# JohnGBaker/ptmcmc

Hardware: AMD Instinct MI355X
Metric: ladder-wide MH steps/sec (D=32 Gaussian, 1024 temps) (higher is better)
Workload: dtype f64

## Files before the change

include/ptm_engine.h:

```cpp
#ifndef PTM_ENGINE_H
#define PTM_ENGINE_H

#include <stddef.h>
#include <stdint.h>

#ifdef __cplusplus
extern "C" {
#endif

#define PTM_ABI_VERSION 3

typedef struct ptm_engine ptm_engine;

#define PTM_COUNT_MAX 2147483647

typedef enum {
  PTM_OK = 0,
  PTM_ERR_INVALID = -1,
  PTM_ERR_UNSUPPORTED = -2,
  PTM_ERR_HIP = -3,
  PTM_ERR_NO_DEVICE = -4,
  PTM_ERR_FAR_MOVE = -5,
  PTM_ERR_CALLBACK = -6
} ptm_status;
// ... 94 lines not shown

int ptm_copy_llike(ptm_engine* e, int first_local_rung, int n_rungs, void* dst_dev);
int ptm_llike_device_ptr(ptm_engine* e, void** dev_ptr);
int ptm_exchange_decide(ptm_engine* e, const void* ll_below_dev, const void* ll_above_dev, int halo_rungs, void* send_up_dev,
                        void* send_down_dev);
int ptm_exchange_decide_gathered(ptm_engine* e, const void* ll_all_dev, const void* lp_all_dev, void* send_up_dev, void* send_down_dev);
int ptm_set_shard_map(ptm_engine* e, int n_shards, const int32_t* rung_counts, int halo_rungs);
int ptm_exchange_redo_count(ptm_engine* e, int* n_ladders);
int ptm_exchange_redo(ptm_engine* e, const void* ll_all_dev, const void* lp_all_dev, void* send_up_dev, void* send_down_dev);
int ptm_copy_lprior(ptm_engine* e, int first_local_rung, int n_rungs, void* dst_dev);
int ptm_exchange_finish_and_sweep(ptm_engine* e, const void* recv_from_below_dev, const void* recv_from_above_dev);
int ptm_exchange_install(ptm_engine* e, const void* recv_from_below_dev, const void* recv_from_above_dev);
int ptm_sweep_rungs(ptm_engine* e, int first_local_rung, int n_rungs, int closes_step);
int ptm_exchange_buffer_doubles(ptm_engine* e);
int ptm_exchange_row_capacity(ptm_engine* e);

#define PTM_SHARD_ID_BYTES 128
int ptm_shard_unique_id(void* id_out);
int ptm_shard_init(ptm_engine* e, const void* id, int rank, int world, const int32_t* rung_counts, int halo_rungs);
int ptm_shard_step(ptm_engine* e, int n);
int ptm_shard_finalize(ptm_engine* e);

enum {
  PTM_ARR_LLIKE = 0,
  PTM_ARR_LPRIOR = 1,
  PTM_ARR_LPOST = 2,
  PTM_ARR_NTRIES = 3,
  PTM_ARR_NACCEPT = 4,
  PTM_ARR_LAST_TYPE = 5,
  PTM_ARR_NHIST = 6,
  PTM_ARR_NSIZE = 7,
  PTM_ARR_ROW_LABELS = 8
};
int ptm_get_states(ptm_engine* e, double* X);
int ptm_get_array(ptm_engine* e, int which, void* out);
int ptm_get_swap_counts(ptm_engine* e, int64_t* tries, int64_t* accepts);
int ptm_get_last_swaps(ptm_engine* e, int32_t* pairs, int32_t* accepted);
int ptm_batch_begin(ptm_engine* e);
int ptm_batch_end(ptm_engine* e);
int ptm_restore(ptm_engine* e, const double* X, const double* llike, const int32_t* ntries, const int32_t* naccept,
                const int32_t* last_type, const int64_t* nhist, uint64_t step_count, const int64_t* swap_tries,
                const int64_t* swap_accepts);
int ptm_max_swaps_per_step(ptm_engine* e);
int ptm_get_history(ptm_engine* e, double* X, double* llike, double* lprior, int32_t* meta);
int ptm_get_history_invtemps(ptm_engine* e, double* beta);
int ptm_get_history_chains(ptm_engine* e, int chain_begin, int chain_count, double* X, double* llike, double* lprior, int32_t* meta, double* invtemps);
int ptm_set_history(ptm_engine* e, const double* X, const double* llike, const double* lprior, const int32_t* meta,
                    const double* invtemps);
int ptm_set_map(ptm_engine* e, const double* X, const double* lpost, const double* llike, const double* lprior);
int ptm_get_map(ptm_engine* e, double* X, double* lpost, double* llike, double* lprior);
uint64_t ptm_step_count(ptm_engine* e);

int ptm_timer_start(ptm_engine* e);
int ptm_timer_stop(ptm_engine* e, float* elapsed_ms);
int ptm_get_kernel_times(ptm_engine* e, float* ms, int capacity, int* count);
const char* ptm_sweep_kernel_name(ptm_engine* e);
const char* ptm_step_kernel_name(ptm_engine* e);

int ptm_get_ladder_stats(ptm_engine* e, int64_t out[4]);
int ptm_get_counter_sums(ptm_engine* e, int64_t* ntries_sum, int64_t* naccept_sum);
int ptm_get_prefilter_counts(ptm_engine* e, int64_t out[4]);
typedef struct ptm_calibration {
  double copy_GBs, copy_bytes, copy_ms;
  double f64_fma_TFs, fma_ms, sclk_MHz;
  int32_t compute_units, reserved;
} ptm_calibration;
int ptm_calibrate(ptm_engine* e, ptm_calibration* out);

int ptm_ess_windowed(ptm_engine* e, int rung, int nfeat, int width, int every, int burn, double* ess , int32_t* nwin );
int ptm_ess_report(ptm_engine* e, int rung, int nfeat, int width, int every, double esslimit, double* ess , int32_t* length );
int ptm_ess_series_windowed(int device, const double* series, int64_t n, int nseries, int nfeat, int width, int every, int burn, double* ess, int32_t* nwin);
int ptm_ess_series_report(int device, const double* series, int64_t n, int nseries, int nfeat, int width, int every, double esslimit, double* ess, int32_t* length);
int ptm_ess_last_on_device(ptm_engine* e);

int ptm_log_evidence(ptm_engine* e, int ilen, double* log_evidence , double* up ,
                     double* down , int32_t* count );

enum { PTM_FN_LOG = 0, PTM_FN_EXP = 1, PTM_FN_SIN_0_PI = 2, PTM_FN_COS_HPI = 3, PTM_FN_SQRT = 4, PTM_FN_DIV = 5,
       PTM_FN_SQRT_RAW = 6 };
int ptm_debug_eval(int device, int fn, const double* a, const double* b, double* out, int n);
int ptm_debug_philox(int device, uint64_t seed, int tag, uint32_t stream, uint64_t step, uint32_t block, uint32_t out[4]);
int ptm_debug_boxmuller(int device, const uint32_t* k1, const uint32_t* k2, double* z0, double* z1, int n);
int ptm_debug_sqrt_scan(int device, uint64_t* mismatches);
int ptm_dev_alloc(size_t bytes, void** out);
int ptm_dev_free(void* p);
int ptm_dev_copy(void* dst, const void* src, size_t bytes);
int ptm_debug_evaluate(ptm_engine* e, const double* X, int n, int32_t* valid, double* X_enforced, double* lprior,
                       double* llike);

#ifdef __cplusplus
}
#endif
#endif
```

ptmcmc_amd/csrc/ptm_aux_kernels.hpp:

```cpp
#pragma once
#include "ptm_kernels.hpp"
#include "ptm_decide.hpp"

namespace ptm {

constexpr int PART_CHUNK = 16384;
__global__ __launch_bounds__(1024) void partition_kernel(int W, int rung0, int nchunk, unsigned char* __restrict__ touch,
                                                         unsigned int* __restrict__ nhist, int* __restrict__ cidx, int* __restrict__ ccnt,
                                                         const unsigned short* __restrict__ rowof, const unsigned char* __restrict__ pflag,
                                                         int* __restrict__ pidx, int* __restrict__ pcnt) {
  extern __shared__ int plist[];
  __shared__ int wsum[16];
  __shared__ int sbase, stotal;
  const int rl = rung0 + blockIdx.x / nchunk, ch = blockIdx.x % nchunk;
  const bool pre = pflag && pflag[rl];
  int* const lidx = pre ? pidx : cidx;
  int* const lcnt = pre ? pcnt : ccnt;
  const int w0 = ch * PART_CHUNK + threadIdx.x * 16;
  const size_t c0 = (size_t)rl * W + w0;
  uint4 v = make_uint4(0x01010101u, 0x01010101u, 0x01010101u, 0x01010101u);
  const bool in = w0 < W;
  if (in) v = *reinterpret_cast<const uint4*>(touch + c0);
  const unsigned int word[4] = {v.x, v.y, v.z, v.w};
  int mine = 0;
// ... 243 lines not shown
  double *x, *ll, *lp;
  const double *recv_below, *recv_above;
  int *arr_below, *arr_above;
  int* err;
};
__global__ __launch_bounds__(256) void install_kernel(const Install p) {
  const double* msg = blockIdx.y ? p.recv_above : p.recv_below;
  if (!msg) return;
  int* arr = blockIdx.y ? p.arr_above : p.arr_below;
  int n = *reinterpret_cast<const int*>(msg);
  if (n > p.row_cap) n = p.row_cap;
  const int j = blockIdx.x * 16 + (threadIdx.x >> 4), sub = threadIdx.x & 15;
  if (j >= n) return;
  const int DP = p.DP, RD = DP + ROW_EXTRA;
  const double* row = msg + MSG_HDR + (size_t)j * RD;
  const int w = (int)row[DP + 2];
  const int a = (w >= 0 && w < p.W) ? arr[w] : -1;
  if (a < 0) { atomicOr(p.err, 8); return; }
  for (int col = 2 * sub; col < DP; col += 32)
    *reinterpret_cast<d2_t*>(p.x + (size_t)a * DP + col) = *reinterpret_cast<const d2_t*>(row + col);
  if (sub == 0) { p.ll[a] = row[DP]; p.lp[a] = row[DP + 1]; }
}

__global__ void hist_init_kernel(Hist h, int DP, const double* x, const double* ll, const double* lp, const int* naccept,
                                 const int* ntries, const int* last_type, const double* beta, const double* betaC, int W, int r0) {
  const int c = blockIdx.x * blockDim.x + threadIdx.x;
  if (c >= h.HC) return;
  const size_t o = hist_slot(h, 0, c);
  for (int d = 0; d < DP; ++d) h.x[o * DP + d] = x[(size_t)c * DP + d];
  hist_scalars(h, o, 0, ll[c], lp[c], naccept[c], ntries[c], last_type[c], betaC ? betaC[c] : beta[r0 + c / W]);
}
__global__ void hist_beta_fill_kernel(Hist h, const double* beta, int W, int r0) {
  const size_t i = (size_t)blockIdx.x * blockDim.x + threadIdx.x;
  if (i >= (size_t)h.cap * h.HC) return;
  h.beta[i] = beta[r0 + (int)(i % h.HC) / W];
}

__global__ void map_init_kernel(MapT m, int DP, int W, int r0, const double* beta, const double* x, const double* ll, const double* lp) {
  const int c = blockIdx.x * blockDim.x + threadIdx.x;
  if (c >= m.MC) return;
  m.lpost[c] = -1e200;
  const double t = beta[r0 + c / W] * ll[c];
  if (map_try(m, c, lp[c] + t, ll[c], lp[c]))
    for (int d = 0; d < DP; ++d) m.x[(size_t)c * DP + d] = x[(size_t)c * DP + d];
}

__global__ void debug_eval_kernel(int fn, const double* a, const double* b, double* out, int n) {
  const int i = blockIdx.x * blockDim.x + threadIdx.x;
  if (i >= n) return;
  double r = 0;
  switch (fn) {
    case 0: r = dlog(a[i]); break;
    case 1: r = dexp(a[i]); break;
    case 2: r = dsin_0_pi(a[i]); break;
    case 3: r = dcos_hpi(a[i]); break;
    case 4: r = dsqrt(a[i]); break;
    case 5: r = a[i] / b[i]; break;
    case 6: r = __builtin_sqrt(a[i]); break;
  }
  out[i] = r;
}
__global__ void debug_philox_kernel(uint64_t seed, int tag, uint32_t stream, uint64_t step, uint32_t block, uint32_t* out) {
  const u32x4 o = draw_block(seed, tag, stream, step, block);
  out[0] = o.v0; out[1] = o.v1; out[2] = o.v2; out[3] = o.v3;
}
__global__ void debug_boxmuller_kernel(const uint32_t* k1, const uint32_t* k2, double* z0, double* z1, int n) {
  const int i = blockIdx.x * blockDim.x + threadIdx.x;
  if (i >= n) return;
  boxmuller(k1[i], k2[i], (const double*)BM_TABLE, z0[i], z1[i]);
}
__global__ void debug_sqrt_scan_kernel(unsigned long long* mismatches) {
  const uint32_t tid = blockIdx.x * blockDim.x + threadIdx.x;
  const uint32_t stride = gridDim.x * blockDim.x;
  unsigned long long bad = 0, out = 0;
  for (uint64_t k = tid; k < (1ull << 32); k += stride) {
    const double a = bm_neg2log((uint32_t)k, (const double*)BM_TABLE);
    if (bm_sqrt(a) != dsqrt(a)) bad++;
    if (!(a > 0.0 && a < 64.0)) out++;
  }
  if (bad) atomicAdd(mismatches, bad);
  if (out) atomicAdd(mismatches + 1, out);
}

__global__ __launch_bounds__(256) void calib_copy_kernel(const uint4* __restrict__ src, uint4* __restrict__ dst, size_t n16) {
  const size_t stride = (size_t)gridDim.x * blockDim.x;
  for (size_t i = (size_t)blockIdx.x * blockDim.x + threadIdx.x; i < n16; i += stride) dst[i] = src[i];
}
__global__ __launch_bounds__(256) void counter_sums_kernel(const int* __restrict__ ntries, const int* __restrict__ naccept, size_t n, unsigned long long* __restrict__ out) {
  __shared__ unsigned long long sh[2][4];
  unsigned long long t = 0, a = 0;
  const size_t stride = (size_t)gridDim.x * blockDim.x;
  for (size_t i = (size_t)blockIdx.x * blockDim.x + threadIdx.x; i < n; i += stride) { t += (unsigned long long)(long long)ntries[i]; a += (unsigned long long)(long long)naccept[i]; }
#pragma unroll
  for (int o = 32; o > 0; o >>= 1) { t += __shfl_down(t, o); a += __shfl_down(a, o); }
  if ((threadIdx.x & 63) == 0) { sh[0][threadIdx.x >> 6] = t; sh[1][threadIdx.x >> 6] = a; }
  __syncthreads();
  if (threadIdx.x == 0) {
    atomicAdd(out, sh[0][0] + sh[0][1] + sh[0][2] + sh[0][3]);
    atomicAdd(out + 1, sh[1][0] + sh[1][1] + sh[1][2] + sh[1][3]);
  }
}
__global__ __launch_bounds__(256) void calib_fma_kernel(double* __restrict__ out, long long* __restrict__ clk, int iters) {
  double d[8];
  const double e0 = 1.0 - 1e-9 * (threadIdx.x & 7), e1 = 1e-12 * (1 + (threadIdx.x & 3));
#pragma unroll
  for (int i = 0; i < 8; ++i) d[i] = 1.0 + 1e-3 * (threadIdx.x + i);
  __syncthreads();
  const long long c0 = (long long)__builtin_amdgcn_s_memtime(), r0 = (long long)__builtin_amdgcn_s_memrealtime();
  for (int it = 0; it < iters; ++it) {
#pragma unroll
    for (int i = 0; i < 8; ++i) asm volatile("v_fma_f64 %0, %0, %1, %2" : "+v"(d[i]) : "v"(e0), "v"(e1));
  }
  const long long c1 = (long long)__builtin_amdgcn_s_memtime(), r1 = (long long)__builtin_amdgcn_s_memrealtime();
  double r = 0.0;
#pragma unroll
  for (int i = 0; i < 8; ++i) r += d[i];
  if (r == 12345.678) out[0] = r;
  if (threadIdx.x == 0) { clk[2 * blockIdx.x] = c1 - c0; clk[2 * blockIdx.x + 1] = r1 - r0; }
}

}
```

ptmcmc_amd/csrc/ptm_box_prefilter.hpp:

```cpp
#pragma once
#include "ptm_kernels.hpp"
#include "ptm_sweep_plan.hpp"

namespace ptm {

#ifndef PTM_BP_ROWS_AHEAD
#define PTM_BP_ROWS_AHEAD 0
#endif

struct BoxPre {
  int W, Nt, r0, w_off;
  int rung0, nrung;
  int labelled;
  uint64_t seed, step;
  const double* x;
  const double *ll, *lp;
  const double* beta;
  const double* prop_tiles;
  const double* box_row;
  int* ntries;
  const int *pidx, *pcnt;
  int *cidx, *ccnt;
  unsigned long long* counts;
};
// ... 72 lines not shown
  PrefilterSlice sl[EA + 1] = {};
  int m[EA + 1] = {};
  BpRows R[2] = {};
#pragma unroll
  for (int k = 0; k < EA; ++k) { sl[k] = slice_of((int)blockIdx.x + k * G); m[k] = load_entry(sl[k]); }
  if (RA) load_rows(sl[0], m[0], R[0]);
  uint64_t pbits = 0;
  int pmine = 0, pbase = 0;
  size_t plbase = 0;
  auto flush = [&]() {
    if (pbits == 0) return;
    const int base = __builtin_amdgcn_readfirstlane(pbase);
    if ((pbits >> l) & 1ull) p.cidx[plbase + base + __builtin_popcountll(pbits & ((1ull << l) - 1ull))] = pmine;
    pbits = 0;
  };
#define PTM_BP_ARRIVED() __builtin_amdgcn_s_waitcnt(0x0F70)
  PTM_BP_ARRIVED();
  unsigned int seen = 0, settled = 0;
  for (int tile = blockIdx.x; tile < ntiles; tile += G) {
    sl[EA] = slice_of(tile + EA * G);
    m[EA] = load_entry(sl[EA]);
    if (RA) load_rows(sl[1], m[1], R[1]);
    else load_rows(sl[0], m[0], R[0]);
    PTM_BP_STAGE();
    const PrefilterSlice s = sl[0];
    const int mine = m[0], nact = s.nact;
    const int rl = p.rung0 + s.r, rg = p.r0 + rl;
    const size_t lbase = (size_t)rl * p.W;
    const BpRows& T = R[0];
    uint64_t inbox = 0;
    if (nact) {
      const bp_d2 lo0 = box[0], lo1 = box[4], hi0 = box[16], hi1 = box[20];
#pragma unroll
      for (int g = 0; g < 4; ++g) {
        const int wk = __shfl(mine, 16 * g + j, 64) & wmask;
        const uint32_t stream = (uint32_t)(wk + p.w_off) * (uint32_t)p.Nt + (uint32_t)rg;
        const u32x4 o = draw_block(p.seed, TAG_MH, stream, p.step, (uint32_t)(1 + q));
        double z[4];
        boxmuller(o.v0, o.v1, L.bm, z[0], z[1]);
        boxmuller(o.v2, o.v3, L.bm, z[2], z[3]);
        bp_d4 acc = bp_d4{0.0, 0.0, 0.0, 0.0};
#pragma unroll
        for (int k = 0; k < 4; ++k) acc = __builtin_amdgcn_mfma_f64_16x16x4f64(T.ta[k], z[k], acc, 0, 0, 0);
        const double x0 = T.v0[g].x + acc[0], x1 = T.v0[g].y + acc[1], x2 = T.v1[g].x + acc[2], x3 = T.v1[g].y + acc[3];
        const bool ok = !(x0 < lo0.x) & !(x0 > hi0.x) & !(x1 < lo0.y) & !(x1 > hi0.y) & !(x2 < lo1.x) & !(x2 > hi1.x) & !(x3 < lo1.y) & !(x3 > hi1.y);
        uint64_t b = __builtin_amdgcn_ballot_w64(ok);
        b &= b >> 32;
        b &= b >> 16;
        inbox |= (b & 0xFFFFull) << (16 * g);
      }
    }
    PTM_BP_STAGE();
    PTM_BP_ARRIVED();
    if (nact) {
      const int c = (int)lbase + (mine & wmask);
      const double cur_lpost = T.lp + T.beta * T.ll;
      const bool live = l < nact;
      const bool finite = __builtin_fabs(cur_lpost) < __builtin_inf();
      const bool settle = live && finite && ((inbox >> l) & 1ull) == 0;
      const bool keep = live && !settle;
      const uint64_t kbits = __builtin_amdgcn_ballot_w64(keep);
      const int nk = __builtin_popcountll(kbits);
      flush();
      if (settle) (void)__hip_atomic_fetch_add(&p.ntries[c], 1, __ATOMIC_RELAXED, __HIP_MEMORY_SCOPE_AGENT);
      if (nk) {
        pbits = kbits; pmine = mine; plbase = lbase;
        const int rlv = __builtin_amdgcn_mov_dpp(rl, 0xE4, 0xF, 0xF, true);
        if (l == 0) pbase = atomicAdd(&p.ccnt[rlv], nk);
      }
      seen += (unsigned int)nact;
      settled += (unsigned int)(nact - nk);
    }
#pragma unroll
    for (int k = 0; k < EA; ++k) { sl[k] = sl[k + 1]; m[k] = m[k + 1]; }
    if (RA) R[0] = R[1];
  }
  flush();
  if (l == 0 && seen) {
    atomicAdd(p.counts, (unsigned long long)seen);
    if (settled) atomicAdd(p.counts + 1, (unsigned long long)settled);
  }
}

}
```

ptmcmc_amd/csrc/ptm_device_math.hpp:

```cpp
#pragma once
#include <hip/hip_runtime.h>
#include <stdint.h>

#include "ptm_lds_layout.hpp"

namespace ptm {

struct u32x4 { uint32_t v0, v1, v2, v3; };
#ifndef PTM_PHILOX_ROUNDS
#define PTM_PHILOX_ROUNDS 10
#endif

struct philox_state { uint32_t c0, c1, c2, c3, k0, k1; };
__device__ __forceinline__ void philox_round(philox_state& s) {
  const uint64_t p0 = (uint64_t)0xD2511F53u * s.c0;
  const uint64_t p1 = (uint64_t)0xCD9E8D57u * s.c2;
  const uint32_t n0 = (uint32_t)(p1 >> 32) ^ s.c1 ^ s.k0;
  const uint32_t n1 = (uint32_t)p1;
  const uint32_t n2 = (uint32_t)(p0 >> 32) ^ s.c3 ^ s.k1;
  const uint32_t n3 = (uint32_t)p0;
  s.c0 = n0; s.c1 = n1; s.c2 = n2; s.c3 = n3;
  s.k0 += 0x9E3779B9u; s.k1 += 0xBB67AE85u;
}
__device__ __forceinline__ u32x4 philox4x32_10(uint32_t c0, uint32_t c1, uint32_t c2, uint32_t c3, uint32_t k0,
// ... 162 lines not shown
}
__device__ __forceinline__ double draw_copolar(double u, double lo, double hi) {
  const double sl = dsin_hpi(lo), sh = dsin_hpi(hi);
  const double y = sl + u * (sh - sl);
  double a = lo, b = hi;
#pragma unroll 1
  for (int k = 0; k < 64; ++k) {
    const double m = 0.5 * (a + b);
    if (dsin_hpi(m) < y) a = m; else b = m;
  }
  return 0.5 * (a + b);
}
__device__ __forceinline__ double draw_log(double u, double lo, double hi) {
  const double l0 = dlog(lo);
  return dexp(u * (dlog(hi) - l0) + l0);
}

__device__ __forceinline__ double dsqrt(double a) {
  const double g = __builtin_sqrt(a);
  const double r = __builtin_fma(-g, g, a);
  const double gn = __longlong_as_double(__double_as_longlong(g) + (r > 0.0 ? 1 : -1));
  const double t = __builtin_fma(-g, gn, a);
  const bool move = (r > 0.0) ? (t > 0.0) : ((r < 0.0) ? (t <= 0.0) : false);
  const bool ok = (a > 0.0) && (a < __builtin_inf());
  return (ok && move) ? gn : g;
}

#include "ptm_tables.inc"
__device__ __attribute__((aligned(16))) const double BM_TABLE[BM_TABLE_DOUBLES] = {PTM_BMTAB_VALUES, PTM_TRIGTAB_VALUES};

typedef double bm_d2 __attribute__((ext_vector_type(2)));

template <class Tab>
__device__ __forceinline__ double bm_neg2log(uint32_t k, Tab tab) {
  const double M2LN2_HI = -2.0 * 6.93147180369123816490e-01, M2LN2_LO = -2.0 * 1.90821492927058770002e-10;
  const double x = (double)k + 0.5;
  const uint64_t b = (uint64_t)__double_as_longlong(x);
  const uint32_t hi = (uint32_t)(b >> 32);
  const uint32_t idx = (hi >> 12) & 255u;
  const int e = (int)(hi >> 20) - (1023 + 32) + (idx >= (uint32_t)PTM_BMTAB_SPLIT ? 1 : 0);
  const double m = __longlong_as_double((long long)((b & 0x000FFFFFFFFFFFFFull) | 0x3FF0000000000000ull));
  const bm_d2 ra = *reinterpret_cast<const bm_d2*>(tab + 2 * idx);
  const double t = __builtin_fma(m, ra.x, -1.0);
  double q = 1.0 / 3.0;
  q = __builtin_fma(q, t, -0.4);
  q = __builtin_fma(q, t, 0.5);
  q = __builtin_fma(q, t, -2.0 / 3.0);
  q = __builtin_fma(q, t, 1.0);
  const double l = __builtin_fma(t * t, q, -2.0 * t);
  const double dk = (double)e;
  return __builtin_fma(dk, M2LN2_HI, ra.y) + __builtin_fma(dk, M2LN2_LO, l);
}

__device__ __forceinline__ double bm_sqrt(double a) {
  const double y = __builtin_amdgcn_rsq(a);
  double g = a * y;
  double h = 0.5 * y;
  const double r = __builtin_fma(-h, g, 0.5);
  g = __builtin_fma(g, r, g);
  h = __builtin_fma(h, r, h);
  const double d = __builtin_fma(-g, g, a);
  return __builtin_fma(d, h, g);
}

template <class Tab>
__device__ __forceinline__ void boxmuller_finish(double r, uint32_t k2, Tab tab, double& z0, double& z1) {
  const uint32_t idx = (k2 >> 21) & 1023u;
  const bm_d2 sc = *reinterpret_cast<const bm_d2*>(tab + 512 + 2 * idx);
  const double d = __builtin_fma((double)((int)(k2 & 0x1FFFFFu) - (1 << 20)), 1.4629180792671596e-09, 0.5 * 1.4629180792671596e-09);
  const double d2 = d * d;
  const double sd = __builtin_fma(d * d2, __builtin_fma(d2, 1.0 / 120.0, -1.0 / 6.0), d);
  const double cm1 = d2 * __builtin_fma(d2, 1.0 / 24.0, -0.5);
  const double sn = __builtin_fma(sc.y, sd, sc.x * cm1) + sc.x;
  const double cs = __builtin_fma(-sc.x, sd, sc.y * cm1) + sc.y;
  r = __longlong_as_double(__double_as_longlong(r) ^ ((long long)(k2 >> 31) << 63));
  z0 = r * cs;
  z1 = r * sn;
}
template <typename Tab>
__device__ __forceinline__ void boxmuller(uint32_t k1, uint32_t k2, Tab tab, double& z0, double& z1) {
  boxmuller_finish(bm_sqrt(bm_neg2log(k1, tab)), k2, tab, z0, z1);
}

__device__ __forceinline__ double fmod_det(double x, double w) {
  const double q = __builtin_trunc(x / w);
  double r = __builtin_fma(-q, w, x);
  if (x >= 0.0) { if (r < 0.0) r += w; else if (r >= w) r -= w; }
  else          { if (r > 0.0) r -= w; else if (r <= -w) r += w; }
  return r;
}

}
```

ptmcmc_amd/csrc/ptm_engine.hip:

```cpp
#include <hip/hip_runtime.h>

#include <algorithm>
#include <cmath>
#include <cstddef>
#include <cstdarg>
#include <cstdio>
#include <cstring>
#include <functional>
#include <memory>
#include <string>
#include <vector>

#include "../../include/ptm_engine.h"
#include "ptm_aux_kernels.hpp"
#include "ptm_box_prefilter.hpp"
#include "ptm_count_limit.hpp"
#include "ptm_de_mfma_kernel.hpp"
#include "ptm_devlike_kernels.hpp"
#include "ptm_ess_kernels.hpp"
#include "ptm_evidence_kernels.hpp"
#include "ptm_launch.hpp"
#include "ptm_shard_rccl.hpp"

using namespace ptm;
// ... 14 lines not shown
    if (_e != hipSuccess) return fail(PTM_ERR_HIP, "%s failed: %s (%s:%d)", #x, hipGetErrorString(_e), __FILE__, __LINE__); \
  } while (0)

template <class T>
struct PinnedAlloc {
  typedef T value_type;
  PinnedAlloc() {}
  template <class U> PinnedAlloc(const PinnedAlloc<U>&) {}
  T* allocate(size_t n) {
    void* p = nullptr;
    if (hipHostMalloc(&p, n * sizeof(T), hipHostMallocMapped | hipHostMallocCoherent) != hipSuccess) throw std::bad_alloc();
    return (T*)p;
  }
  void deallocate(T* p, size_t) { (void)hipHostFree(p); }
  template <class U> bool operator==(const PinnedAlloc<U>&) const { return true; }
  template <class U> bool operator!=(const PinnedAlloc<U>&) const { return false; }
};
template <class T> using pinned_vector = std::vector<T, PinnedAlloc<T>>;

struct ptm_engine {
  ptm_config cfg;
  int D = 0, DP = 0, Nt = 0, r0 = 0, nloc = 0, W = 0, Nc = 0, ms = 0;
  int device = 0;
  hipStream_t stream = nullptr;
  bool own_stream = false;
  uint64_t step = 0;
  double *xdev = nullptr, *ll = nullptr, *lp = nullptr;
  int *ntries = nullptr, *naccept = nullptr, *last_type = nullptr, *err = nullptr;
  int *arr_below = nullptr, *arr_above = nullptr;
  int *mv_src = nullptr, *mv_dst = nullptr, *mv_n = nullptr;
  unsigned int* nhist = nullptr;
  long long* swap_cnt = nullptr;
  unsigned char* touch = nullptr;
  Hist hist = {0, 0, 0, nullptr, nullptr, nullptr, nullptr, nullptr};
  MapT map = {0, 0, nullptr, nullptr, nullptr, nullptr};
  int* swap_log = nullptr;
  int log_head = 0, log_pending = 0;
  int row_cap = 0;
  int *blo = nullptr, *bhi = nullptr, *ptype = nullptr;
  double *bmin = nullptr, *bmax = nullptr, *plo = nullptr, *phi = nullptr, *pcoef = nullptr;
  double *P2 = nullptr, *mean = nullptr, *beta = nullptr, *prop = nullptr, *prop_tiles = nullptr, *P2_tiles = nullptr, *box_row = nullptr, *onedfrac = nullptr, *mix = nullptr;
  int mix_K = 0;
  bool de_on = false;
  ptm_de_params de = {0, 0, 0, 0};
  int de_init_extra = 0;
  double *de_init = nullptr, *de_hast = nullptr;
  int* de_type = nullptr;
  bool ada_on = false;
  ptm_adaptive_set ada = {0, -1, 0, 0, 0};
  double *ada_leaf = nullptr, *ada_dbl = nullptr;
  int* ada_int = nullptr;
  int prior_member = -1;
  std::vector<char> set_neg;
  double evolve_rate = 0, evolve_cut = -1;
  double *beta_w = nullptr, *betaC = nullptr, *beta_add = nullptr;
  bool betaC_stale = false;
  int has_bounds = 0, origin_valid = 1, all_uniform = 1, has_mean = 0, have_target = 0, have_ladder = 0,
      have_prop = 0, have_state = 0, prop_kind = KIND_DIAG, prop_stride = 0, any_oned = 0, bounds_box = 1;
  double lprior_const = 0, like0 = 0, thresh = 0;
  bool lp_is_const = false;
  std::vector<double> h_beta;
  std::vector<int> h_ptype;
  std::vector<double> h_plo, h_phi;
  ptm_loglike_batch_fn cb = nullptr;
  void* cb_user = nullptr;
  ptm_logprior_batch_fn prior_cb = nullptr;
  void* prior_user = nullptr;
  ptm_propose_batch_fn pcb = nullptr;
  ptm_proposal_result_fn pres = nullptr;
  void* pcb_user = nullptr;
  ptm_loglike_device_fn dfn = nullptr;
  void* dfn_user = nullptr;
  double *dl_x = nullptr, *dl_ll = nullptr;
  bool dl_own_x = false, dl_own_ll = false;
  int32_t* dl_count = nullptr;
  int *dl_rows = nullptr, *dl_chunks = nullptr;
  double *dl_xprop = nullptr, *dl_lprior_new = nullptr, *dl_llike_new = nullptr, *dl_best = nullptr;
  unsigned char* dl_gate = nullptr;
  int *cidx = nullptr, *ccnt = nullptr;
  int *pidx = nullptr, *pcnt = nullptr;
  unsigned char *pf_flag = nullptr, *h_pf_flag = nullptr;
  unsigned long long* pf_counts = nullptr;
  std::vector<double> pf_sigma;
  bool pf_dirty = true;
  int pf_flagged = 0, pf_grid = 0;
  bool touched = false;
  bool compact_step = false;
  unsigned short* rowof = nullptr;
  bool rows_labelled = false;
  bool label_step = false;
  ShardComm* shard = nullptr;
  int* shard_ends = nullptr;
  int nshards = 0, halo_nominal = 0;
  int* redo_flag = nullptr;
  long long redo_total = 0;
  double *pub_x = nullptr, *pub_ll = nullptr, *pub_lp = nullptr;
  int *lad_flags = nullptr, *lad_ctl = nullptr;
  long long* lad_prof = nullptr;
  int lad_capacity[2][32] = {{-1, -1, -1, -1, -1, -1, -1, -1, -1, -1, -1, -1, -1, -1, -1, -1, -1, -1, -1, -1, -1, -1, -1, -1, -1, -1, -1, -1, -1, -1, -1, -1},
                             {-1, -1, -1, -1, -1, -1, -1, -1, -1, -1, -1, -1, -1, -1, -1, -1, -1, -1, -1, -1, -1, -1, -1, -1, -1, -1, -1, -1, -1, -1, -1, -1}};
  long long ladder_launches = 0, ladder_whole_steps = 0;
  struct LadLaunch { int seq; uint64_t step_before; int nsteps; int log_head_before; };
  std::vector<LadLaunch> lad_log;
  int lad_deferred = 0;
  int lad_seq = 0;
  bool lad_disabled = false;
  long long ladder_fallbacks = 0;
  hipEvent_t lad_event = nullptr;
  unsigned int nhist_pending = 0;
  CountHorizon horizon;
  bool step_booked = false;
  int steps_prepaid = 0;
  double* hastings = nullptr;
  int* htype = nullptr;
  unsigned char *hvalid = nullptr, *acc_out = nullptr;
  pinned_vector<double> h_rows, h_hast;
  pinned_vector<int> h_type;
  pinned_vector<unsigned char> h_valid, h_touch, h_acc;
  std::vector<double> p_xcur, p_xprop, p_hast;
  std::vector<int32_t> p_rung, p_walker, p_type, p_valid, p_acc;
  std::vector<size_t> p_pick;
  double *xprop = nullptr, *lprior_new = nullptr, *llike_new = nullptr;
  pinned_vector<unsigned char> fetch_arena;
  size_t fetch_used = 0;
  int fetch_depth = 0;
  std::vector<std::function<void()>> fetch_after;
  std::vector<std::shared_ptr<std::vector<unsigned char>>> fetch_big;
  std::vector<std::pair<unsigned char*, size_t>> host_blocks;
  bool shared_handover = false, hist_on_host = false;
  unsigned char* gate = nullptr;
  pinned_vector<double> h_xprop, h_llnew;
  std::vector<double> h_batch, h_llbatch;
  unsigned char* h_gate = nullptr;
  unsigned long long *sums = nullptr, *h_sums = nullptr;
  void* ess_ws = nullptr;
  size_t ess_ws_bytes = 0;
  int ess_on_device = 0;
  hipEvent_t t0 = nullptr, t1 = nullptr;
  std::vector<hipEvent_t> kev;
  size_t kev_used = 0;
  std::string kname;
};

#include <mutex>
static std::mutex g_lad_mutex;
static ptm_engine* g_lad_last = nullptr;

static int round_dp(int D) {
  if (D <= 4) return 4;
  if (D <= 8) return 8;
  if (D <= 16) return 16;
  if (D <= 32) return 32;
  if (D <= 64) return 64;
  if (D <= 128) return 128;
  if (D <= 256) return 256;
  if (D <= 512) return 512;
  return 1024;
}

template <class T>
static int dalloc(T** p, size_t n) {
  HIPCHK(hipMalloc((void**)p, (n ? n : 1) * sizeof(T)));
  return PTM_OK;
}
static hipError_t copy_unless_shared(void* dst, const void* src, size_t bytes, hipMemcpyKind kind, hipStream_t s) {
  if (dst == src) return hipSuccess;
// ... 162 lines not shown
  e->all_uniform = 0;
  HIPCHK(hipEventCreate(&e->t0));
  HIPCHK(hipEventCreate(&e->t1));
  HIPCHK(hipStreamSynchronize(e->stream));
  return PTM_OK;
}

template <class T>
static int halloc(ptm_engine* e, T** p, size_t n) {
  void* h = nullptr;
  const size_t bytes = (n ? n : 1) * sizeof(T);
  HIPCHK(hipHostMalloc(&h, bytes, hipHostMallocMapped | hipHostMallocCoherent));
  e->host_blocks.push_back(std::make_pair((unsigned char*)h, bytes));
  *p = (T*)h;
  return PTM_OK;
}

static const size_t FETCH_ARENA = (size_t)4 << 20;
static int fetch_flush(ptm_engine* e) {
  HIPCHK(hipStreamSynchronize(e->stream));
  for (auto& f : e->fetch_after) f();
  e->fetch_after.clear(); e->fetch_big.clear(); e->fetch_used = 0;
  return PTM_OK;
}
static int fetch_raw(ptm_engine* e, const void* dev, size_t bytes, const unsigned char** staged) {
  for (const auto& b : e->host_blocks)
    if ((const unsigned char*)dev >= b.first && (const unsigned char*)dev < b.first + b.second) {
      *staged = (const unsigned char*)dev;
      return PTM_OK;
    }
  if (e->fetch_arena.empty()) e->fetch_arena.resize(FETCH_ARENA);
  const size_t need = (bytes + 63) & ~(size_t)63;
  if (need > FETCH_ARENA / 2 || e->fetch_used + need > FETCH_ARENA) {
    auto buf = std::make_shared<std::vector<unsigned char>>(bytes);
    HIPCHK(hipStreamSynchronize(e->stream));
    HIPCHK(hipMemcpy(buf->data(), dev, bytes, hipMemcpyDeviceToHost));
    e->fetch_big.push_back(buf);
    *staged = buf->data();
    return PTM_OK;
  }
  unsigned char* at = e->fetch_arena.data() + e->fetch_used;
  HIPCHK(hipMemcpyAsync(at, dev, bytes, hipMemcpyDeviceToHost, e->stream));
  e->fetch_used += need;
  *staged = at;
  return PTM_OK;
}
static int fetch(ptm_engine* e, const void* dev, size_t bytes, const unsigned char** staged) {
  const int rc = fetch_raw(e, dev, bytes, staged);
  if (rc) { e->fetch_after.clear(); e->fetch_big.clear(); e->fetch_used = 0; }
  return rc;
}
static int fetch_done(ptm_engine* e) { return e->fetch_depth > 0 ? PTM_OK : fetch_flush(e); }
#define SETTLE(e) do { if (e) { const int _rc = ladder_settle(e); if (_rc) return _rc; } } while (0)
#define NO_BATCH(e, name) do { if ((e) && (e)->fetch_depth > 0) return fail(PTM_ERR_INVALID, name " between ptm_batch_begin and ptm_batch_end (only reads go there)"); } while (0)
#define FETCH(ptr, dev, bytes) do { int _rc = fetch(e, (dev), (bytes), &(ptr)); if (_rc) return _rc; } while (0)

extern "C" int ptm_batch_begin(ptm_engine* e) {
  SETTLE(e);
  if (!e) return fail(PTM_ERR_INVALID, "null engine");
  e->fetch_depth++;
  return PTM_OK;
}
extern "C" int ptm_batch_end(ptm_engine* e) {
  if (!e) return fail(PTM_ERR_INVALID, "null engine");
  if (e->fetch_depth <= 0) return fail(PTM_ERR_INVALID, "ptm_batch_end without ptm_batch_begin");
  if (--e->fetch_depth > 0) return PTM_OK;
  return fetch_flush(e);
}

extern "C" int ptm_engine_destroy(ptm_engine* e) {
  if (!e) return PTM_OK;
  (void)ptm_shard_finalize(e);
  (void)hipStreamSynchronize(e->stream);
  {
    std::lock_guard<std::mutex> lock(g_lad_mutex);
    if (g_lad_last == e) g_lad_last = nullptr;
  }
  if (e->lad_event) (void)hipEventDestroy(e->lad_event);
  if (e->shared_handover) e->xprop = e->llike_new = nullptr, e->hastings = nullptr, e->htype = nullptr, e->hvalid = e->acc_out = nullptr;
  if (e->hist_on_host) e->hist.x = e->hist.ll = e->hist.lp = e->hist.beta = nullptr, e->hist.meta = nullptr;
  for (auto& b : e->host_blocks) (void)hipHostFree(b.first);
  void* ptrs[] = {e->xdev, e->rowof, e->ll, e->lp, e->ntries, e->naccept, e->last_type, e->arr_below, e->arr_above, e->mv_src, e->mv_dst, e->mv_n,
                  e->err, e->nhist, e->swap_cnt, e->touch, e->swap_log, e->hist.x, e->hist.ll, e->hist.lp, e->hist.meta, e->map.lpost, e->map.ll, e->map.lp, e->map.x, e->blo,
                  e->bhi, e->ptype, e->bmin, e->bmax, e->plo, e->phi, e->pcoef, e->P2, e->mean, e->beta, e->prop, e->prop_tiles, e->P2_tiles, e->box_row, e->onedfrac, e->mix, e->beta_w, e->betaC, e->beta_add, e->hist.beta, e->xprop, e->lprior_new, e->llike_new, e->hastings, e->htype, e->hvalid, e->acc_out, e->cidx, e->ccnt, e->pidx, e->pcnt, e->pf_flag, e->pf_counts,
                  e->pub_x, e->lad_flags, e->lad_prof, e->shard_ends, e->redo_flag, e->sums, e->de_init, e->de_hast, e->de_type,
                  e->ada_leaf, e->ada_dbl, e->ada_int, e->dl_own_x ? e->dl_x : nullptr, e->dl_own_ll ? e->dl_ll : nullptr, e->dl_count, e->dl_rows, e->dl_chunks, e->dl_xprop,
                  e->dl_lprior_new, e->dl_llike_new, e->dl_best, e->ess_ws};
  for (void* p : ptrs)
    if (p) (void)hipFree(p);
  if (e->h_sums) (void)hipHostFree(e->h_sums);
  if (e->h_pf_flag) (void)hipHostFree(e->h_pf_flag);
  for (hipEvent_t ev : e->kev) (void)hipEventDestroy(ev);
  if (e->t0) (void)hipEventDestroy(e->t0);
  if (e->t1) (void)hipEventDestroy(e->t1);
  if (e->own_stream) (void)hipStreamDestroy(e->stream);
  delete e;
  return PTM_OK;
}

extern "C" int ptm_set_bounds(ptm_engine* e, const int32_t* lo, const int32_t* hi, const double* xmin, const double* xmax) {
  SETTLE(e);
  if (!e || !lo || !hi || !xmin || !xmax) return fail(PTM_ERR_INVALID, "null argument");
  int rc;
  const int D = e->D;
  e->has_bounds = 0;
  e->bounds_box = 1;
  for (int d = 0; d < D; ++d) {
    if (lo[d] < 0 || lo[d] > 3 || hi[d] < 0 || hi[d] > 3) return fail(PTM_ERR_INVALID, "bad boundary type in dimension %d", d);
    if (lo[d] != PTM_BOUND_OPEN || hi[d] != PTM_BOUND_OPEN) e->has_bounds = 1;
    if ((lo[d] != PTM_BOUND_OPEN && lo[d] != PTM_BOUND_LIMIT) || (hi[d] != PTM_BOUND_OPEN && hi[d] != PTM_BOUND_LIMIT)) e->bounds_box = 0;
  }
  e->origin_valid = 1;
  for (int d = 0; d < D; ++d) {
    const bool lw = lo[d] == PTM_BOUND_WRAP, hw = hi[d] == PTM_BOUND_WRAP;
    if (lw != hw) { e->origin_valid = 0; break; }
    if (lw) { if (xmax[d] - xmin[d] <= 0) { e->origin_valid = 0; break; } continue; }
    if (lo[d] == PTM_BOUND_REFLECT && hi[d] == PTM_BOUND_REFLECT) { if (xmax[d] - xmin[d] <= 0) { e->origin_valid = 0; break; } continue; }
    double z = 0.0;
    if (lo[d] == PTM_BOUND_REFLECT && z < xmin[d]) z = xmin[d] + (xmin[d] - z);
    else if (hi[d] == PTM_BOUND_REFLECT && z > xmax[d]) z = xmax[d] - (z - xmax[d]);
    if (lo[d] == PTM_BOUND_LIMIT && z < xmin[d]) { e->origin_valid = 0; break; }
    if (hi[d] == PTM_BOUND_LIMIT && z > xmax[d]) { e->origin_valid = 0; break; }
  }
  if ((rc = upload(e->blo, lo, D, e->stream)) || (rc = upload(e->bhi, hi, D, e->stream)) ||
      (rc = upload(e->bmin, xmin, D, e->stream)) || (rc = upload(e->bmax, xmax, D, e->stream)))
    return rc;
  return PTM_OK;
}

static inline size_t host_row_pos(size_t DP, size_t d);
extern "C" int ptm_set_prior(ptm_engine* e, const int32_t* types, const double* c, const double* h) {
  SETTLE(e);
  if (!e || !types || !c || !h) return fail(PTM_ERR_INVALID, "null argument");
  const int D = e->D;
  std::vector<double> lo(D), hi(D), coef(D);
  std::vector<int> ty(D);
  e->all_uniform = 1;
  double prod = 1;
  for (int d = 0; d < D; ++d) {
    ty[d] = types[d];
    switch (types[d]) {
      case PTM_PRIOR_FLAT: lo[d] = -INFINITY; hi[d] = INFINITY; coef[d] = 1; e->all_uniform = 0; break;
      case PTM_PRIOR_UNIFORM: lo[d] = c[d] - h[d]; hi[d] = c[d] + h[d]; coef[d] = 1 / (hi[d] - lo[d]); prod *= coef[d]; break;
      case PTM_PRIOR_GAUSSIAN: lo[d] = c[d]; hi[d] = h[d]; coef[d] = 0; e->all_uniform = 0; break;
      case PTM_PRIOR_POLAR: {
        double a = c[d] - h[d], b = c[d] + h[d];
        lo[d] = a; hi[d] = b;
        if (a < 0) a = 0;
        if (b > M_PI) b = M_PI;
        coef[d] = -std::cos(b) + std::cos(a);
        e->all_uniform = 0;
        break;
      }
      case PTM_PRIOR_COPOLAR: {
        double a = c[d] - h[d], b = c[d] + h[d];
        lo[d] = a; hi[d] = b;
        if (a < -M_PI / 2) a = -M_PI / 2;
        if (b > M_PI / 2) b = M_PI / 2;
        coef[d] = std::sin(b) - std::sin(a);
        e->all_uniform = 0;
        break;
      }
      case PTM_PRIOR_LOG:
        if (c[d] <= 0 || h[d] <= 1) return fail(PTM_ERR_INVALID, "log prior needs center>0 and halfwidth>1 (dimension %d)", d);
        lo[d] = c[d] / h[d]; hi[d] = c[d] * h[d]; coef[d] = std::log(hi[d]) - std::log(lo[d]);
        e->all_uniform = 0;
        break;
      default: return fail(PTM_ERR_INVALID, "unknown prior type %d in dimension %d", types[d], d);
    }
  }
  e->lprior_const = std::log(prod);
  e->pf_dirty = true;
  e->lp_is_const = false;
  for (int d = 0; d < D; ++d) { e->h_ptype[d] = ty[d]; e->h_plo[d] = lo[d]; e->h_phi[d] = hi[d]; }
// ... 240 lines not shown

extern "C" int ptm_set_invtemps(ptm_engine* e, const double* beta) {
  SETTLE(e);
  NO_BATCH(e, "ptm_set_invtemps");
  if (!e || !beta) return fail(PTM_ERR_INVALID, "null argument");
  if (!e->beta_w) return fail(PTM_ERR_INVALID, "per-ladder temperatures exist only once the ladders evolve (ptm_set_evolve_temps)");
  HIPCHK(hipStreamSynchronize(e->stream));
  HIPCHK(hipMemcpy(e->beta_w, beta, (size_t)e->W * e->Nt * 8, hipMemcpyHostToDevice));
  return launch_beta_transpose(e);
}

extern "C" int ptm_set_proposals(ptm_engine* e, int kind, const double* factors, const double* one_d_frac) {
  SETTLE(e);
  if (!e || !factors) return fail(PTM_ERR_INVALID, "null argument");
  const int D = e->D, DP = e->DP, nloc = e->nloc;
  int stride;
  std::vector<double> packed;
  if (kind == PTM_PROP_DIAG) {
    stride = DP;
    packed.assign((size_t)nloc * stride, 0.0);
    for (int r = 0; r < nloc; ++r)
      for (int d = 0; d < D; ++d) packed[(size_t)r * stride + d] = factors[(size_t)r * D + d];
  } else if (kind == PTM_PROP_DENSE || kind == PTM_PROP_LOWER) {
    stride = DP * DP;
    packed.assign((size_t)nloc * stride, 0.0);
    for (int r = 0; r < nloc; ++r)
      for (int i = 0; i < D; ++i)
        for (int j = 0; j < D; ++j) packed[(size_t)r * stride + (size_t)j * DP + i] = factors[(size_t)r * D * D + (size_t)i * D + j];
    if (kind == PTM_PROP_LOWER)
      for (int r = 0; r < nloc; ++r)
        for (int i = 0; i < D; ++i)
          for (int j = i + 1; j < D; ++j)
            if (factors[(size_t)r * D * D + (size_t)i * D + j] != 0.0)
              return fail(PTM_ERR_INVALID, "PTM_PROP_LOWER factor of local rung %d has a non-zero above the diagonal", r);
  } else {
    return fail(PTM_ERR_INVALID, "unknown proposal kind %d", kind);
  }
  if (e->prop) { HIPCHK(hipStreamSynchronize(e->stream)); HIPCHK(hipFree(e->prop)); e->prop = nullptr; }
  if (e->prop_tiles) { HIPCHK(hipFree(e->prop_tiles)); e->prop_tiles = nullptr; }
  int rc;
  if ((rc = dalloc(&e->prop, packed.size())) || (rc = upload(e->prop, packed.data(), packed.size(), e->stream))) return rc;
  if (DP == 32) {
    std::vector<double> tiles((size_t)nloc * 16 * 64, 0.0);
    for (int r = 0; r < nloc; ++r)
      for (int t = 0; t < 16; ++t) {
        const int rt = t & 1, sl = (t >> 1) & 3, hb = t >> 3;
        for (int k = 0; k < 4; ++k)
          for (int i = 0; i < 16; ++i) {
            const int row = 16 * rt + i, col = 16 * hb + 4 * k + sl;
            if (row < D && col < D)
              tiles[((size_t)r * 16 + t) * 64 + 16 * k + i] =
                  kind == PTM_PROP_DIAG ? (row == col ? factors[(size_t)r * D + row] : 0.0) : factors[(size_t)r * D * D + (size_t)row * D + col];
          }
      }
    if ((rc = dalloc(&e->prop_tiles, tiles.size())) || (rc = upload(e->prop_tiles, tiles.data(), tiles.size(), e->stream))) return rc;
  }
  if (DP == 64 || DP == 128) {
    const int NT = DP / 16, ntile = NT * NT * 4;
    std::vector<double> tiles((size_t)nloc * ntile * 64, 0.0);
    for (int r = 0; r < nloc; ++r)
      for (int t = 0; t < ntile; ++t) {
        const int rt = t % NT, sl = (t / NT) & 3, hb = t / (4 * NT);
        for (int k = 0; k < 4; ++k)
          for (int i = 0; i < 16; ++i) {
            const int row = 16 * rt + i, col = 16 * hb + 4 * k + sl;
            if (row < D && col < D)
              tiles[((size_t)r * ntile + t) * 64 + 16 * k + i] =
                  kind == PTM_PROP_DIAG ? (row == col ? factors[(size_t)r * D + row] : 0.0) : factors[(size_t)r * D * D + (size_t)row * D + col];
          }
      }
    if ((rc = dalloc(&e->prop_tiles, tiles.size())) || (rc = upload(e->prop_tiles, tiles.data(), tiles.size(), e->stream))) return rc;
  }
  std::vector<double> f(nloc, 0.0);
  e->any_oned = 0;
  if (one_d_frac)
    for (int r = 0; r < nloc; ++r) {
      if (one_d_frac[r] < 0 || one_d_frac[r] > 1) return fail(PTM_ERR_INVALID, "oneDfrac must be in [0,1]");
      f[r] = one_d_frac[r];
      if (f[r] > 0) e->any_oned = 1;
    }
  if ((rc = upload(e->onedfrac, f.data(), (size_t)nloc, e->stream))) return rc;
  e->prop_kind = kind; e->prop_stride = stride; e->have_prop = 1;
  e->pf_sigma.assign((size_t)nloc * PREFILTER_DIMS, 0.0);
  for (int r = 0; r < nloc; ++r) prefilter_sigmas(kind == PTM_PROP_DIAG, factors + (size_t)r * (kind == PTM_PROP_DIAG ? D : D * D), D, &e->pf_sigma[(size_t)r * PREFILTER_DIMS]);
  e->pf_dirty = true;
  return PTM_OK;
}

static int ada_off(ptm_engine* e) {
  e->ada_on = false;
  if (!e->ada_leaf && !e->ada_dbl && !e->ada_int) return PTM_OK;
  HIPCHK(hipStreamSynchronize(e->stream));
  if (e->ada_leaf) HIPCHK(hipFree(e->ada_leaf));
  if (e->ada_dbl) HIPCHK(hipFree(e->ada_dbl));
  if (e->ada_int) HIPCHK(hipFree(e->ada_int));
  e->ada_leaf = e->ada_dbl = nullptr;
  e->ada_int = nullptr;
  return PTM_OK;
}

extern "C" int ptm_set_proposal_mixture(ptm_engine* e, int K, const double* cum_shares, const double* scales, const double* one_d_fracs) {
  SETTLE(e);
  if (!e) return fail(PTM_ERR_INVALID, "null engine");
  if (!e->have_prop) return fail(PTM_ERR_INVALID, "set the base proposals first (ptm_set_proposals)");
  if (K < 0 || K > 64) return fail(PTM_ERR_INVALID, "mixture size must be in 0..64");
  if (e->mix) { HIPCHK(hipStreamSynchronize(e->stream)); HIPCHK(hipFree(e->mix)); e->mix = nullptr; }
  e->mix_K = 0;
  e->prior_member = -1; e->set_neg.clear();
  { const int rc = ada_off(e); if (rc) return rc; }
  if (K == 0) return PTM_OK;
  if (!cum_shares || !scales || !one_d_fracs) return fail(PTM_ERR_INVALID, "null argument");
  const int nloc = e->nloc;
  std::vector<double> t((size_t)nloc * K * 3);
  int oned = 0;
  for (int r = 0; r < nloc; ++r)
    for (int k = 0; k < K; ++k) {
      const size_t i = (size_t)r * K + k;
      if (k > 0 && cum_shares[i] < cum_shares[i - 1]) return fail(PTM_ERR_INVALID, "cumulative shares must not decrease (rung %d)", r);
      if (one_d_fracs[i] < 0 || one_d_fracs[i] > 1) return fail(PTM_ERR_INVALID, "oneDfrac must be in [0,1]");
      t[3 * i] = cum_shares[i]; t[3 * i + 1] = scales[i]; t[3 * i + 2] = one_d_fracs[i];
      if (one_d_fracs[i] > 0) oned = 1;
    }
  int rc;
  if ((rc = dalloc(&e->mix, t.size())) || (rc = upload(e->mix, t.data(), t.size(), e->stream))) return rc;
  e->mix_K = K;
  e->set_neg.assign((size_t)K, 0);
  for (int r = 0; r < nloc; ++r)
    for (int k = 0; k < K; ++k)
      if (scales[(size_t)r * K + k] < 0) e->set_neg[k] = 1;
  if (oned) e->any_oned = 1;
  return PTM_OK;
}

static int ada_check_state(const ptm_adaptive_set& a, size_t Nc, const double* w, const double* th, const int32_t* bits, const int32_t* cnt) {
  if (!w || !th || !bits || !cnt) return fail(PTM_ERR_INVALID, "null argument");
  const int L = a.K + a.K_inner;
  for (size_t c = 0; c < Nc; ++c)
    for (int b = 0; b < 2; ++b) {
      const int first = b ? a.K : 0, n = b ? a.K_inner : a.K;
      const int32_t bv = bits[c * 2 + b], cv = cnt[c * 2 + b];
      if (bv < 0 || (n < 31 && bv >= (1 << n)) || cv < 0)
        return fail(PTM_ERR_INVALID, "adaptive set: repeat bits name members of the set only and outcome counts are >= 0 (chain %zu)", c);
      if (n == 0) continue;
      double sum = 0.0, prev = 0.0;
      for (int k = 0; k < n; ++k) {
        const double wk = w[c * L + first + k], tk = th[c * L + first + k];
        if (!std::isfinite(wk) || wk < 0) return fail(PTM_ERR_INVALID, "adaptive set: weights must be finite and >= 0 (chain %zu)", c);
        if (!(tk >= prev && tk <= 1.0)) return fail(PTM_ERR_INVALID, "adaptive set: thresholds must not decrease and lie in [0, 1] (chain %zu)", c);
        sum += wk;
        prev = tk;
      }
      if (!(sum > 0)) return fail(PTM_ERR_INVALID, "adaptive set: the weights of a set must have a positive sum (chain %zu)", c);
      if (prev != 1.0) return fail(PTM_ERR_INVALID, "adaptive set: the last threshold of a set must be exactly 1 (chain %zu)", c);
    }
  return PTM_OK;
}
static void ada_to_soa(size_t Nc, int L, const double* w, const double* th, const int32_t* bits, const int32_t* cnt, std::vector<double>& dbl, std::vector<int>& in) {
  dbl.assign(2 * (size_t)L * Nc, 0.0);
  in.assign(4 * Nc, 0);
  for (size_t c = 0; c < Nc; ++c) {
    for (int k = 0; k < L; ++k) { dbl[(size_t)k * Nc + c] = w[c * L + k]; dbl[((size_t)L + k) * Nc + c] = th[c * L + k]; }
    for (int b = 0; b < 2; ++b) { in[(size_t)b * Nc + c] = bits[c * 2 + b]; in[(size_t)(2 + b) * Nc + c] = cnt[c * 2 + b]; }
  }
}

extern "C" int ptm_set_proposal_adaptive(ptm_engine* e, const ptm_adaptive_set* a, const double* scales, const double* one_d_fracs, const double* weights,
                                         const double* thresholds, const int32_t* repeat_bits, const int32_t* outcomes) {
// ... 124 lines not shown
  SETTLE(e);
  if (!e) return fail(PTM_ERR_INVALID, "null engine");
  NO_BATCH(e, "ptm_set_proposal_de");
  HIPCHK(hipStreamSynchronize(e->stream));
  if (e->de_init) { HIPCHK(hipFree(e->de_init)); e->de_init = nullptr; }
  e->de_on = false; e->de_init_extra = 0;
  if (!q) return PTM_OK;
  if (e->DP > 128) return fail(PTM_ERR_UNSUPPORTED, "differential evolution on the device is built for up to 128 dimensions; above, draw it on the host (ptm_set_proposal_callback)");
  if (e->nloc != e->Nt)
    return fail(PTM_ERR_UNSUPPORTED, "differential evolution draws from EVERY rung's saved history, and a rung shard cannot record its top rung's: the row that "
                                     "rung holds between two exchanges of one step sits in the shard above (error bit 16).  Split the population by walkers "
                                     "(whole ladders per GPU: walker_begin) or draw on the host (ptm_set_proposal_callback)");
  if (e->hist.rungs != e->nloc || e->hist.cap < 2)
    return fail(PTM_ERR_INVALID, "differential evolution draws from every rung's saved history: create the engine with history_rungs = rung_count and a "
                                 "history_capacity that holds every row of the run");
  if (e->pcb) return fail(PTM_ERR_INVALID, "host-side proposals are set (ptm_set_proposal_callback): they replace every device proposal");
  if (!(q->snooker >= 0 && q->snooker <= 1) || !(q->gamma_one_frac >= 0 && q->gamma_one_frac <= 1) || !(q->reduce_gamma > 0) ||
      !(q->ignore_frac >= 0 && q->ignore_frac < 1) || n_init_extra < 0 || (n_init_extra > 0 && !init_rows))
    return fail(PTM_ERR_INVALID, "differential evolution: snooker and gamma_one_frac in [0, 1], reduce_gamma > 0, ignore_frac in [0, 1), init rows given");
  int rc;
  if (n_init_extra > 0) {
    const size_t Nc = e->Nc, D = e->D, DP = e->DP;
    std::vector<double> img((size_t)n_init_extra * Nc * DP, 0.0);
    for (size_t k = 0; k < (size_t)n_init_extra; ++k)
      for (size_t c = 0; c < Nc; ++c)
        for (size_t d = 0; d < D; ++d) img[(k * Nc + c) * DP + host_row_pos(DP, d)] = init_rows[(k * Nc + c) * D + d];
    if ((rc = dalloc(&e->de_init, img.size()))) return rc;
    HIPCHK(hipMemcpy(e->de_init, img.data(), img.size() * 8, hipMemcpyHostToDevice));
  }
  if (!e->de_hast && ((rc = dalloc(&e->de_hast, (size_t)e->Nc)) || (rc = dalloc(&e->de_type, (size_t)e->Nc)))) return rc;
  e->de = *q;
  e->de_init_extra = n_init_extra;
  e->de_on = true;
  return PTM_OK;
}

extern "C" int ptm_set_proposal_rung(ptm_engine* e, int local_rung, const double* factor, double one_d_frac) {
  SETTLE(e);
  if (!e || !factor) return fail(PTM_ERR_INVALID, "null argument");
  if (!e->have_prop) return fail(PTM_ERR_INVALID, "set all proposals first (ptm_set_proposals)");
  if (local_rung < 0 || local_rung >= e->nloc) return fail(PTM_ERR_INVALID, "rung out of the shard");
  const int D = e->D, DP = e->DP, kind = e->prop_kind == KIND_DIAG ? PTM_PROP_DIAG : (e->prop_kind == KIND_LOWER ? PTM_PROP_LOWER : PTM_PROP_DENSE);
  std::vector<double> packed((size_t)e->prop_stride, 0.0);
  if (kind == PTM_PROP_DIAG) {
    for (int d = 0; d < D; ++d) packed[d] = factor[d];
  } else {
    for (int i = 0; i < D; ++i)
      for (int j = 0; j < D; ++j) {
        if (kind == PTM_PROP_LOWER && j > i && factor[(size_t)i * D + j] != 0.0)
          return fail(PTM_ERR_INVALID, "PTM_PROP_LOWER factor has a non-zero above the diagonal");
        packed[(size_t)j * DP + i] = factor[(size_t)i * D + j];
      }
  }
  int rc;
  if ((rc = upload(e->prop + (size_t)local_rung * e->prop_stride, packed.data(), packed.size(), e->stream))) return rc;
  if (DP == 32) {
    std::vector<double> tiles(16 * 64, 0.0);
    for (int t = 0; t < 16; ++t) {
      const int rt = t & 1, sl = (t >> 1) & 3, hb = t >> 3;
      for (int k = 0; k < 4; ++k)
        for (int i = 0; i < 16; ++i) {
          const int row = 16 * rt + i, col = 16 * hb + 4 * k + sl;
          if (row < D && col < D)
            tiles[(size_t)t * 64 + 16 * k + i] = kind == PTM_PROP_DIAG ? (row == col ? factor[row] : 0.0) : factor[(size_t)row * D + col];
        }
    }
    if ((rc = upload(e->prop_tiles + (size_t)local_rung * 16 * 64, tiles.data(), tiles.size(), e->stream))) return rc;
  }
  if (DP == 64 || DP == 128) {
    const int NT = DP / 16, ntile = NT * NT * 4;
    std::vector<double> tiles((size_t)ntile * 64, 0.0);
    for (int t = 0; t < ntile; ++t) {
      const int rt = t % NT, sl = (t / NT) & 3, hb = t / (4 * NT);
      for (int k = 0; k < 4; ++k)
        for (int i = 0; i < 16; ++i) {
          const int row = 16 * rt + i, col = 16 * hb + 4 * k + sl;
          if (row < D && col < D)
            tiles[(size_t)t * 64 + 16 * k + i] = kind == PTM_PROP_DIAG ? (row == col ? factor[row] : 0.0) : factor[(size_t)row * D + col];
        }
    }
    if ((rc = upload(e->prop_tiles + (size_t)local_rung * ntile * 64, tiles.data(), tiles.size(), e->stream))) return rc;
  }
  prefilter_sigmas(kind == PTM_PROP_DIAG, factor, D, &e->pf_sigma[(size_t)local_rung * PREFILTER_DIMS]);
  e->pf_dirty = true;
  if (one_d_frac >= 0) {
    if (one_d_frac > 1) return fail(PTM_ERR_INVALID, "oneDfrac must be in [0,1]");
    if ((rc = upload(e->onedfrac + local_rung, &one_d_frac, 1, e->stream))) return rc;
    if (one_d_frac > 0) e->any_oned = 1;
  }
  return PTM_OK;
}

static Dev make_dev(ptm_engine* e, bool labelled = false) {
  Dev p;
  memset(&p, 0, sizeof p);
  p.D = e->D; p.DP = e->DP; p.Nt = e->Nt; p.r0 = e->r0; p.nloc = e->nloc; p.W = e->W; p.Nc = e->Nc; p.w_off = e->cfg.walker_begin;
  p.seed = e->cfg.seed; p.step = e->step; p.add_every_n = e->cfg.add_every_n; p.min_prior = e->cfg.min_prior;
  p.has_bounds = e->has_bounds; p.origin_valid = e->origin_valid; p.bounds_box = e->bounds_box;
  p.blo = e->blo; p.bhi = e->bhi; p.bmin = e->bmin; p.bmax = e->bmax;
  p.all_uniform = e->all_uniform; p.lprior_const = e->lprior_const;
  p.ptype = e->ptype; p.plo = e->plo; p.phi = e->phi; p.pcoef = e->pcoef;
  p.P2 = e->P2; p.mean = e->mean; p.has_mean = e->has_mean; p.like0 = e->like0;
  p.beta = e->beta; p.prop = e->prop; p.prop_tiles = e->prop_tiles; p.P2_tiles = e->P2_tiles; p.box_row = e->box_row; p.onedfrac = e->onedfrac; p.prop_stride = e->prop_stride; p.any_oned = e->any_oned;
  p.mix_K = e->mix_K; p.mix = e->mix;
  p.de_on = e->de_on ? 1 : 0; p.de_init_extra = e->de_init_extra; p.de_init = e->de_init; p.de_hast = e->de_hast; p.de_type = e->de_type;
  p.de_snooker = e->de.snooker; p.de_gamma_one = e->de.gamma_one_frac; p.de_gamma_div = e->de.reduce_gamma; p.de_ignore = e->de.ignore_frac;
  p.de_gamma_std = e->de_on ? 1.68 / std::sqrt((double)e->D) / e->de.reduce_gamma : 0.0;
  p.prior_k = e->prior_member + 1;
  p.betaC = e->betaC; p.beta_add = e->beta_add; p.beta_w = e->beta_w;
  p.x = labelled ? e->xdev : xrows(e); p.ll = e->ll; p.lp = e->lp;
  p.ntries = e->ntries; p.naccept = e->naccept; p.last_type = e->last_type; p.nhist = e->nhist;
  p.touch = e->touch; p.err = e->err;
  p.hist = e->hist;
  p.map = e->map;
  p.c_begin = 0; p.c_end = e->Nc;
  p.host_prop = e->pcb ? 1 : 0; p.hastings = e->hastings; p.htype = e->htype; p.hvalid = e->hvalid; p.acc_out = e->acc_out;
  return p;
}

static AdaArgs make_ada(const ptm_engine* e) {
  AdaArgs a;
  memset(&a, 0, sizeof a);
  if (!e->ada_on) return a;
  const size_t L = (size_t)e->ada.K + e->ada.K_inner, Nc = e->Nc;
  a.K = e->ada.K; a.nested = e->ada.nested; a.Ki = e->ada.K_inner; a.rate = e->ada.rate; a.rate_in = e->ada.rate_inner;
  a.leaf = e->ada_leaf; a.w = e->ada_dbl; a.th = e->ada_dbl + L * Nc; a.bits = e->ada_int; a.cnt = e->ada_int + 2 * Nc;
  return a;
}

const DpLaunch* ptm::dp_launch(int DP) {
  switch (DP) {
    case 4: return &dp_launch_4;
    case 8: return &dp_launch_8;
    case 16: return &dp_launch_16;
    case 32: return &dp_launch_32;
    case 64: return &dp_launch_64;
    case 128: return &dp_launch_128;
    case 256: return &dp_launch_256;
    case 512: return &dp_launch_512;
    case 1024: return &dp_launch_1024;
  }
  return nullptr;
}

static inline bool user_like(const ptm_engine* e) { return e->cb != nullptr || e->dfn != nullptr; }

static SweepFacts sweep_facts(const ptm_engine* e, long long chains, bool touched) {
  SweepFacts f;
  memset(&f, 0, sizeof f);
  f.DP = e->DP; f.W = e->W; f.chains = chains; f.nloc = e->nloc;
  f.kind = e->prop_kind == PTM_PROP_DIAG ? PLAN_DIAG : (e->prop_kind == PTM_PROP_LOWER ? PLAN_LOWER : PLAN_DENSE);
  f.has_bounds = e->has_bounds; f.bounds_box = e->bounds_box; f.all_uniform = e->all_uniform; f.has_mean = e->has_mean; f.any_oned = e->any_oned;
  f.mix_K = e->mix_K;
  f.evolving = e->betaC != nullptr; f.tracked = e->hist.rungs || e->map.rungs;
  f.user_like = user_like(e); f.host_prop = e->pcb != nullptr; f.ada = e->ada_on;
  f.de = e->de_on || e->prior_member >= 0;
  f.mode = f.user_like ? 1 : 0;
  f.touched = touched;
  f.prior_draw = e->prior_member >= 0; f.history = e->hist.rungs > 0 && e->hist.rungs == e->nloc;
  return f;
}
static SweepPlan sweep_plan(const ptm_engine* e, long long chains, bool touched) { return plan_sweep(sweep_facts(e, chains, touched), sweep_env()); }
static SweepPlan step_sweep_plan(const ptm_engine* e) { return sweep_plan(e, e->Nc, true); }
static bool de_mfma_sweep(const ptm_engine* e, long long chains) { return e->de_on && de_mfma_applies(sweep_facts(e, chains, true), sweep_env()); }

static bool lean_ev_sweeps(const ptm_engine* e) { return reads_ladder_major_beta(step_sweep_plan(e)); }
// ... 96 lines not shown
  NO_BATCH(e, "ptm_set_target_device");
  if (e->prior_cb) return fail(PTM_ERR_UNSUPPORTED, "a host-evaluated prior with a device likelihood is not built (ptm_set_prior_callback)");
  if (e->pcb) return fail(PTM_ERR_UNSUPPORTED, "host-side proposals with a device likelihood are not built (ptm_set_proposal_callback)");
  if (e->nloc != e->Nt) return fail(PTM_ERR_UNSUPPORTED, "a device likelihood on a rung shard is not built: split such a population by walkers");
  const size_t Nc = e->Nc, D = e->D, DP = e->DP;
  int rc;
  if (!e->dl_count &&
      ((rc = dalloc(&e->dl_count, 1)) || (rc = dalloc(&e->dl_rows, Nc)) || (rc = dalloc(&e->dl_chunks, (Nc + DL_CHUNK - 1) / DL_CHUNK)) ||
       (rc = dalloc(&e->dl_xprop, Nc * DP)) || (rc = dalloc(&e->dl_gate, Nc)) || (rc = dalloc(&e->dl_lprior_new, Nc)) ||
       (rc = dalloc(&e->dl_llike_new, Nc)) || (rc = dalloc(&e->dl_best, D + 1))))
    return rc;
  if (x_batch_dev) {
    if (e->dl_own_x && e->dl_x) { HIPCHK(hipStreamSynchronize(e->stream)); (void)hipFree(e->dl_x); }
    e->dl_x = x_batch_dev; e->dl_own_x = false;
  } else if (!e->dl_own_x) {
    e->dl_x = nullptr;
    if ((rc = dalloc(&e->dl_x, Nc * D))) return rc;
    e->dl_own_x = true;
  }
  if (llike_batch_dev) {
    if (e->dl_own_ll && e->dl_ll) { HIPCHK(hipStreamSynchronize(e->stream)); (void)hipFree(e->dl_ll); }
    e->dl_ll = llike_batch_dev; e->dl_own_ll = false;
  } else if (!e->dl_own_ll) {
    e->dl_ll = nullptr;
    if ((rc = dalloc(&e->dl_ll, Nc))) return rc;
    e->dl_own_ll = true;
  }
  HIPCHK(hipMemsetAsync(e->dl_gate, 0, Nc, e->stream));
  if ((rc = devlike_reset_best(e))) return rc;
  e->dfn = fn; e->dfn_user = user;
  e->cb = nullptr;
  e->have_target = 1;
  return PTM_OK;
}

extern "C" int ptm_target_device_rows(ptm_engine* e) {
  if (!e) return fail(PTM_ERR_INVALID, "null engine");
  return e->Nc;
}

extern "C" int ptm_get_best_evaluated(ptm_engine* e, double* lpost, double* x) {
  if (!e || !lpost) return fail(PTM_ERR_INVALID, "null argument");
  SETTLE(e);
  NO_BATCH(e, "ptm_get_best_evaluated");
  if (!e->dl_best) return fail(PTM_ERR_INVALID, "no device likelihood set (ptm_set_target_device)");
  std::vector<double> b((size_t)e->D + 1);
  HIPCHK(hipMemcpyAsync(b.data(), e->dl_best, b.size() * 8, hipMemcpyDeviceToHost, e->stream));
  HIPCHK(hipStreamSynchronize(e->stream));
  *lpost = b[0];
  if (x) memcpy(x, b.data() + 1, (size_t)e->D * 8);
  return PTM_OK;
}

static int devlike_debug(ptm_engine* e, const double* X, int n, double* llike) {
  const size_t Nc = e->Nc, D = e->D;
  std::vector<double> rows(Nc * D);
  for (size_t k0 = 0; k0 < (size_t)n; k0 += Nc) {
    const size_t m = std::min(Nc, (size_t)n - k0);
    for (size_t k = 0; k < Nc; ++k) memcpy(&rows[k * D], X + (k0 + (k < m ? k : 0)) * D, D * 8);
    const int32_t cnt = (int32_t)m;
    HIPCHK(hipMemcpyAsync(e->dl_x, rows.data(), Nc * D * 8, hipMemcpyHostToDevice, e->stream));
    HIPCHK(hipMemcpyAsync(e->dl_count, &cnt, 4, hipMemcpyHostToDevice, e->stream));
    e->dfn(e->dfn_user, (void*)e->stream, (int)Nc, (int)D, e->dl_x, e->dl_count, e->dl_ll);
    HIPCHK(hipMemcpyAsync(llike + k0, e->dl_ll, m * 8, hipMemcpyDeviceToHost, e->stream));
    HIPCHK(hipStreamSynchronize(e->stream));
  }
  return PTM_OK;
}

#define NO_DEVLIKE(e, name) do { if ((e) && (e)->dfn) return fail(PTM_ERR_UNSUPPORTED, name " with a device likelihood is not built (rung-sharded steps)"); } while (0)

static int prefilter_flags(ptm_engine* e) {
  const int nd = e->D < PREFILTER_DIMS ? e->D : PREFILTER_DIMS;
  double width[PREFILTER_DIMS];
  for (int d = 0; d < nd; ++d) width[d] = e->h_phi[d] - e->h_plo[d];
  if (!e->h_pf_flag) HIPCHK(hipHostMalloc((void**)&e->h_pf_flag, (size_t)e->nloc, hipHostMallocDefault));
  unsigned char* fl = e->h_pf_flag;
  e->pf_flagged = 0;
  for (int r = 0; r < e->nloc; ++r) {
    fl[r] = (e->pf_sigma.size() == (size_t)e->nloc * PREFILTER_DIMS && prefilter_flag(&e->pf_sigma[(size_t)r * PREFILTER_DIMS], width, nd, sweep_env().prefilter)) ? 1 : 0;
    e->pf_flagged += fl[r];
  }
  HIPCHK(hipMemcpyAsync(e->pf_flag, fl, (size_t)e->nloc, hipMemcpyHostToDevice, e->stream));
  e->pf_dirty = false;
  return PTM_OK;
}

static int launch_sweep(ptm_engine* e, int rung0 = 0, int nr = -1, bool last = true) {
  const bool labelled = e->label_step;
  e->label_step = false;
  Dev p = make_dev(e, labelled);
  if (nr < 0) nr = e->nloc - rung0;
  if (rung0 < 0 || nr < 0 || rung0 + nr > e->nloc) return fail(PTM_ERR_INVALID, "rung range out of the shard");
  p.c_begin = rung0 * e->W; p.c_end = (rung0 + nr) * e->W;
  if ((user_like(e) || e->pcb) && (rung0 != 0 || nr != e->nloc)) return fail(PTM_ERR_UNSUPPORTED, "partial sweeps with a user likelihood (host or device) or host-side proposals are not built");
  auto close_step = [&]() {
    e->step += 1; e->touched = false; e->step_booked = false;
    if (e->compact_step) { e->nhist_pending += 1; e->compact_step = false; }
  };
  if (nr == 0) { if (last) close_step(); return PTM_OK; }
  hipEvent_t ev0 = nullptr, ev1 = nullptr;
  if (e->cfg.time_kernels) {
    if (e->kev_used + 2 > e->kev.size()) {
      for (int k = 0; k < 2; ++k) { hipEvent_t ev; HIPCHK(hipEventCreate(&ev)); e->kev.push_back(ev); }
    }
    ev0 = e->kev[e->kev_used]; ev1 = e->kev[e->kev_used + 1];
    e->kev_used += 2;
  }
  const SweepPlan plan = sweep_plan(e, p.c_end - p.c_begin, e->touched);
  if (e->betaC_stale && !reads_ladder_major_beta(plan)) { int rc = ensure_betaC(e); if (rc) return rc; }
  const bool compact = plan.compacted;
  if (labelled && !(compact && rung0 == 0 && nr == e->nloc)) return fail(PTM_ERR_HIP, "internal: a labelled exchange phase without its compacted sweep");
  if (!compact) { int rc = flush_nhist(e); if (rc) return rc; }
  if (compact) {
    if (!e->cidx) { int rc; if ((rc = dalloc(&e->cidx, (size_t)e->Nc)) || (rc = dalloc(&e->ccnt, (size_t)e->nloc))) return rc; }
    HIPCHK(hipMemsetAsync(e->ccnt + rung0, 0, (size_t)nr * sizeof(int), e->stream));
    bool pre = plan.prefilter;
    if (pre) {
      if (!e->pidx) {
        int rc;
        if ((rc = dalloc(&e->pidx, (size_t)e->Nc)) || (rc = dalloc(&e->pcnt, (size_t)e->nloc)) || (rc = dalloc(&e->pf_flag, (size_t)e->nloc)) || (rc = dalloc(&e->pf_counts, 2))) return rc;
        HIPCHK(hipMemsetAsync(e->pf_counts, 0, 16, e->stream));
        e->pf_dirty = true;
      }
      if (e->pf_dirty) { int rc = prefilter_flags(e); if (rc) return rc; }
      pre = e->pf_flagged > 0;
      if (pre) HIPCHK(hipMemsetAsync(e->pcnt + rung0, 0, (size_t)nr * sizeof(int), e->stream));
    }
    const int nchunk = (e->W + PART_CHUNK - 1) / PART_CHUNK;
    hipLaunchKernelGGL(partition_kernel, dim3((unsigned)((size_t)nr * nchunk)), dim3(1024), (size_t)PART_CHUNK * sizeof(int), e->stream, e->W, rung0, nchunk, e->touch, e->nhist,
                       e->cidx, e->ccnt, labelled ? (const unsigned short*)e->rowof : nullptr, pre ? (const unsigned char*)e->pf_flag : nullptr, e->pidx, e->pcnt);
    e->compact_step = true;
    HIPCHK(hipGetLastError());
    if (pre) {
      BoxPre b;
      memset(&b, 0, sizeof b);
      b.W = e->W; b.Nt = e->Nt; b.r0 = e->r0; b.w_off = e->cfg.walker_begin; b.rung0 = rung0; b.nrung = nr; b.labelled = labelled ? 1 : 0;
      b.seed = e->cfg.seed; b.step = e->step;
      b.x = p.x; b.ll = e->ll; b.lp = e->lp; b.beta = e->beta; b.prop_tiles = e->prop_tiles; b.box_row = e->box_row; b.ntries = e->ntries;
      b.pidx = e->pidx; b.pcnt = e->pcnt; b.cidx = e->cidx; b.ccnt = e->ccnt; b.counts = e->pf_counts;
      const size_t lds = BoxPreLds(nullptr, nr).bytes;
      if (!e->pf_grid) {
        int per_cu = 0, dev = 0;
        hipDeviceProp_t pr;
        if (hipOccupancyMaxActiveBlocksPerMultiprocessor(&per_cu, (const void*)box_prefilter_kernel, 256, BoxPreLds(nullptr, e->nloc).bytes) != hipSuccess || per_cu <= 0) { (void)hipGetLastError(); per_cu = 2; }
        HIPCHK(hipGetDevice(&dev));
        HIPCHK(hipGetDeviceProperties(&pr, dev));
        e->pf_grid = per_cu * (pr.multiProcessorCount > 0 ? pr.multiProcessorCount : 256);
        const int cap = sweep_env().prefilter_grid;
        if (cap > 0 && cap < e->pf_grid) e->pf_grid = cap;
      }
      const long long tiles = (long long)nr * ((e->W + 255) / 256);
      hipLaunchKernelGGL(box_prefilter_kernel, dim3((unsigned)(tiles < e->pf_grid ? tiles : e->pf_grid)), dim3(256), lds, e->stream, b);
      HIPCHK(hipGetLastError());
    }
    p.cidx = e->cidx; p.ccnt = e->ccnt; p.cidx_slot = labelled ? 1 : 0;
  }
  if (ev0) HIPCHK(hipEventRecord(ev0, e->stream));
  const AdaArgs ada = make_ada(e);
  const DpLaunch* dl = dp_launch(e->DP);
  if (!dl) return fail(PTM_ERR_UNSUPPORTED, "dim > 1024 is not built");
  const bool de_mfma = de_mfma_sweep(e, p.c_end - p.c_begin);
  if (de_mfma && (compact || plan.family == FAM_MFMA32)) return fail(PTM_ERR_HIP, "internal: differential evolution on the matrix cores beside a matrix-core plan");
  auto launch = [&](const Dev& q) {
    if (de_mfma) return launch_de_mfma32(q, e->prop_kind == PTM_PROP_DENSE ? KIND_DENSE : KIND_LOWER, e->betaC != nullptr, e->stream);
    return dl->sweep(q, plan, e->stream, ada);
  };

  size_t npick = 0;
  if (e->pcb) {
    const size_t Nc = e->Nc, D = e->D, DP = e->DP;
    HIPCHK(hipMemcpyAsync(e->h_rows.data(), xrows(e), Nc * DP * 8, hipMemcpyDeviceToHost, e->stream));
    HIPCHK(hipMemcpyAsync(e->h_touch.data(), e->touch, Nc, hipMemcpyDeviceToHost, e->stream));
    HIPCHK(hipStreamSynchronize(e->stream));
    e->p_pick.clear();
    for (size_t c = 0; c < Nc; ++c)
      if (!e->h_touch[c]) e->p_pick.push_back(c);
    npick = e->p_pick.size();
    e->p_xcur.resize(npick * D); e->p_xprop.assign(npick * D, 0.0); e->p_hast.assign(npick, 0.0);
    e->p_rung.resize(npick); e->p_walker.resize(npick); e->p_type.assign(npick, 0); e->p_valid.assign(npick, 1);
    for (size_t k = 0; k < npick; ++k) {
      const size_t c = e->p_pick[k];
      for (size_t d = 0; d < D; ++d) e->p_xcur[k * D + d] = e->h_rows[c * DP + host_row_pos(DP, d)];
      e->p_rung[k] = e->r0 + (int)(c / e->W); e->p_walker[k] = e->cfg.walker_begin + (int)(c % e->W);
    }
    if (npick)
      e->pcb(e->pcb_user, (int)npick, (int)D, e->p_xcur.data(), e->p_rung.data(), e->p_walker.data(), e->step, e->p_xprop.data(),
             e->p_hast.data(), e->p_type.data(), e->p_valid.data());
    for (size_t k = 0; k < npick; ++k) {
      const size_t c = e->p_pick[k];
      for (size_t d = 0; d < DP; ++d) e->h_xprop[c * DP + d] = 0.0;
      for (size_t d = 0; d < D; ++d) e->h_xprop[c * DP + host_row_pos(DP, d)] = e->p_xprop[k * D + d];
      e->h_hast[c] = e->p_hast[k]; e->h_type[c] = e->p_type[k]; e->h_valid[c] = e->p_valid[k] ? 1 : 0;
    }
    HIPCHK(copy_unless_shared(e->xprop, e->h_xprop.data(), Nc * DP * 8, hipMemcpyHostToDevice, e->stream));
    HIPCHK(copy_unless_shared(e->hastings, e->h_hast.data(), Nc * 8, hipMemcpyHostToDevice, e->stream));
    HIPCHK(copy_unless_shared(e->htype, e->h_type.data(), Nc * 4, hipMemcpyHostToDevice, e->stream));
    HIPCHK(copy_unless_shared(e->hvalid, e->h_valid.data(), Nc, hipMemcpyHostToDevice, e->stream));
    p.xprop = e->xprop; p.lprior_new = e->lprior_new; p.gate = e->gate; p.llike_new = e->llike_new;
  }
  if (e->dfn) {
    p.xprop = e->dl_xprop; p.lprior_new = e->dl_lprior_new; p.gate = e->dl_gate; p.llike_new = e->dl_llike_new;
    p.mode = 1;
    HIPCHK(launch(p));
    { const int rc = devlike_eval(e, e->dl_gate, 2, 2, e->dl_xprop, xrows(e), e->dl_llike_new, nullptr, e->dl_lprior_new, true); if (rc) return rc; }
    p.mode = 2;
    HIPCHK(launch(p));
  } else if (!e->cb) {
    HIPCHK(launch(p));
  } else {
    const size_t Nc = e->Nc, DP = e->DP;
    p.xprop = e->xprop; p.lprior_new = e->lprior_new; p.gate = e->gate; p.llike_new = e->llike_new;
    p.mode = 1;
    HIPCHK(launch(p));
    { const int rc = callback_host_part(e); if (rc) return rc; }
    p.mode = 2;
    HIPCHK(launch(p));
  }
  if (e->pcb && e->pres && npick) {
    HIPCHK(copy_unless_shared(e->h_acc.data(), e->acc_out, (size_t)e->Nc, hipMemcpyDeviceToHost, e->stream));
    HIPCHK(hipStreamSynchronize(e->stream));
    e->p_acc.resize(npick);
    for (size_t k = 0; k < npick; ++k) e->p_acc[k] = e->h_acc[e->p_pick[k]] == 1 ? 1 : 0;
    e->pres(e->pcb_user, (int)npick, e->p_rung.data(), e->p_walker.data(), e->p_acc.data());
  }
  if (ev1) HIPCHK(hipEventRecord(ev1, e->stream));
  if (last) close_step();
  return PTM_OK;
}

static int fold_swap_log(ptm_engine* e) {
  if (!e->log_pending) return PTM_OK;
  const int first = ((e->log_head - e->log_pending) % PTM_LOG_RING + PTM_LOG_RING) % PTM_LOG_RING;
  if (e->Nt > 1) {
    hipLaunchKernelGGL(fold_swap_log_kernel, dim3(e->W), dim3(256), (size_t)2 * (e->Nt - 1) * sizeof(int), e->stream, e->swap_log, e->swap_cnt,
                       e->W, e->ms, e->Nt, e->r0, e->r0 + e->nloc, first, e->log_pending);
// ... 1736 lines not shown
  else hipLaunchKernelGGL(evidence_ratio_kernel<false>, grid, dim3(EVID_THREADS), 0, e->stream, src, d_up, d_dn, d_cnt, d_flag);
  HIPCHK(hipGetLastError());
  hipLaunchKernelGGL(evidence_total_kernel, dim3((unsigned)((W + EVID_THREADS - 1) / EVID_THREADS)), dim3(EVID_THREADS), 0, e->stream, src, d_up, d_dn, d_ev);
  HIPCHK(hipGetLastError());
  int flag = 0;
  HIPCHK(hipMemcpyAsync(&flag, d_flag, 4, hipMemcpyDeviceToHost, e->stream));
  HIPCHK(hipStreamSynchronize(e->stream));
  if (flag) return fail(PTM_ERR_INVALID, "ptm_log_evidence: history_capacity must hold the evidence window (%d rows hold less than the last %d steps of every chain)", e->hist.cap, ilen);
  HIPCHK(hipMemcpyAsync(log_evidence, d_ev, W * 8, hipMemcpyDeviceToHost, e->stream));
  if (up) HIPCHK(hipMemcpyAsync(up, d_up, np * 8, hipMemcpyDeviceToHost, e->stream));
  if (down) HIPCHK(hipMemcpyAsync(down, d_dn, np * 8, hipMemcpyDeviceToHost, e->stream));
  if (count) HIPCHK(hipMemcpyAsync(count, d_cnt, Nc * 4, hipMemcpyDeviceToHost, e->stream));
  HIPCHK(hipStreamSynchronize(e->stream));
  return PTM_OK;
}

extern "C" int ptm_debug_eval(int device, int fn, const double* a, const double* b, double* out, int n) {
  int rc = need_device();
  if (rc) return rc;
  if (device >= 0) HIPCHK(hipSetDevice(device));
  double *da = nullptr, *db = nullptr, *dout = nullptr;
  HIPCHK(hipMalloc((void**)&da, (size_t)n * 8));
  HIPCHK(hipMalloc((void**)&db, (size_t)n * 8));
  HIPCHK(hipMalloc((void**)&dout, (size_t)n * 8));
  HIPCHK(hipMemcpy(da, a, (size_t)n * 8, hipMemcpyHostToDevice));
  HIPCHK(hipMemcpy(db, b ? b : a, (size_t)n * 8, hipMemcpyHostToDevice));
  hipLaunchKernelGGL(debug_eval_kernel, dim3((n + 255) / 256), dim3(256), 0, 0, fn, da, db, dout, n);
  HIPCHK(hipGetLastError());
  HIPCHK(hipMemcpy(out, dout, (size_t)n * 8, hipMemcpyDeviceToHost));
  (void)hipFree(da); (void)hipFree(db); (void)hipFree(dout);
  return PTM_OK;
}

extern "C" int ptm_debug_philox(int device, uint64_t seed, int tag, uint32_t stream, uint64_t step, uint32_t block, uint32_t out[4]) {
  int rc = need_device();
  if (rc) return rc;
  if (device >= 0) HIPCHK(hipSetDevice(device));
  uint32_t* d = nullptr;
  HIPCHK(hipMalloc((void**)&d, 16));
  hipLaunchKernelGGL(debug_philox_kernel, dim3(1), dim3(1), 0, 0, seed, tag, stream, step, block, d);
  HIPCHK(hipGetLastError());
  HIPCHK(hipMemcpy(out, d, 16, hipMemcpyDeviceToHost));
  (void)hipFree(d);
  return PTM_OK;
}

extern "C" int ptm_debug_boxmuller(int device, const uint32_t* k1, const uint32_t* k2, double* z0, double* z1, int n) {
  int rc = need_device();
  if (rc) return rc;
  if (device >= 0) HIPCHK(hipSetDevice(device));
  uint32_t *d1 = nullptr, *d2 = nullptr;
  double *o0 = nullptr, *o1 = nullptr;
  HIPCHK(hipMalloc((void**)&d1, (size_t)n * 4));
  HIPCHK(hipMalloc((void**)&d2, (size_t)n * 4));
  HIPCHK(hipMalloc((void**)&o0, (size_t)n * 8));
  HIPCHK(hipMalloc((void**)&o1, (size_t)n * 8));
  HIPCHK(hipMemcpy(d1, k1, (size_t)n * 4, hipMemcpyHostToDevice));
  HIPCHK(hipMemcpy(d2, k2, (size_t)n * 4, hipMemcpyHostToDevice));
  hipLaunchKernelGGL(debug_boxmuller_kernel, dim3((n + 255) / 256), dim3(256), 0, 0, d1, d2, o0, o1, n);
  HIPCHK(hipGetLastError());
  HIPCHK(hipMemcpy(z0, o0, (size_t)n * 8, hipMemcpyDeviceToHost));
  HIPCHK(hipMemcpy(z1, o1, (size_t)n * 8, hipMemcpyDeviceToHost));
  (void)hipFree(d1); (void)hipFree(d2); (void)hipFree(o0); (void)hipFree(o1);
  return PTM_OK;
}

extern "C" int ptm_debug_sqrt_scan(int device, uint64_t* mismatches) {
  int rc = need_device();
  if (rc) return rc;
  if (!mismatches) return fail(PTM_ERR_INVALID, "null argument");
  if (device >= 0) HIPCHK(hipSetDevice(device));
  unsigned long long* d = nullptr;
  HIPCHK(hipMalloc((void**)&d, 16));
  HIPCHK(hipMemset(d, 0, 16));
  hipLaunchKernelGGL(debug_sqrt_scan_kernel, dim3(256 * 16), dim3(256), 0, 0, d);
  HIPCHK(hipGetLastError());
  unsigned long long v[2] = {0, 0};
  HIPCHK(hipMemcpy(v, d, 16, hipMemcpyDeviceToHost));
  (void)hipFree(d);
  *mismatches = v[0] + v[1];
  return PTM_OK;
}

extern "C" int ptm_debug_evaluate(ptm_engine* e, const double* X, int n, int32_t* valid, double* Xe, double* lprior, double* llike) {
  if (!e || !X || n < 1) return fail(PTM_ERR_INVALID, "bad argument");
  const size_t D = e->D, DP = e->DP;
  std::vector<double> rows = pad_rows(X, (size_t)n, D, DP);
  double *dx = nullptr, *dlp = nullptr, *dll = nullptr;
  int* dv = nullptr;
  HIPCHK(hipMalloc((void**)&dx, (size_t)n * DP * 8));
  HIPCHK(hipMalloc((void**)&dlp, (size_t)n * 8));
  HIPCHK(hipMalloc((void**)&dll, (size_t)n * 8));
  HIPCHK(hipMalloc((void**)&dv, (size_t)n * 4));
  HIPCHK(hipMemcpy(dx, rows.data(), (size_t)n * DP * 8, hipMemcpyHostToDevice));
  int rc = run_eval(e, n, dx, dv, dlp, dll, (e->have_target && !user_like(e)) ? 1 : 0);
  if (rc) return rc;
  HIPCHK(hipStreamSynchronize(e->stream));
  HIPCHK(hipMemcpy(rows.data(), dx, (size_t)n * DP * 8, hipMemcpyDeviceToHost));
  if (Xe) unpad_rows(rows, (size_t)n, D, DP, Xe);
  if (valid) HIPCHK(hipMemcpy(valid, dv, (size_t)n * 4, hipMemcpyDeviceToHost));
  if (lprior) HIPCHK(hipMemcpy(lprior, dlp, (size_t)n * 8, hipMemcpyDeviceToHost));
  if (llike && e->have_target && !user_like(e)) HIPCHK(hipMemcpy(llike, dll, (size_t)n * 8, hipMemcpyDeviceToHost));
  if (llike && e->dfn) {
    std::vector<double> xe((size_t)n * D);
    unpad_rows(rows, (size_t)n, D, DP, xe.data());
    if ((rc = devlike_debug(e, xe.data(), n, llike))) return rc;
  }
  (void)hipFree(dx); (void)hipFree(dlp); (void)hipFree(dll); (void)hipFree(dv);
  return PTM_OK;
}
```

ptmcmc_amd/csrc/ptm_lds_layout.hpp:

```cpp
#pragma once
#include <stddef.h>
#include <stdint.h>

#if defined(__HIPCC__)
#define PTM_LDS_FN __host__ __device__ __forceinline__
#else
#define PTM_LDS_FN inline
#endif

namespace ptm {

constexpr int BM_TABLE_DOUBLES = 512 + 2048;
constexpr int MVCAP = 256;
constexpr int M64_P2_TILES = 40;
constexpr int M128_P2_TILES = 144;
constexpr int M128_THREADS = 512;

struct LdsCarve {
  unsigned char* cur;
  size_t off, bytes;
  bool live;
  PTM_LDS_FN explicit LdsCarve(void* b, size_t o = 0) : cur(static_cast<unsigned char*>(b)), off(o), bytes(o), live(true) {}
  template <class T>
  PTM_LDS_FN void take(T*& p, const char* , int n) {
// ... 82 lines not shown
    c.take(olist, "olist", msp);
    c.take(opos, "opos", msp);
    c.take(ti, "ti", msp);
    c.take(tdep, "tdep", msp);
    c.take(tacc, "tacc", ms8);
    c.tail(evolve && (evb || cut));
    const size_t p0_at = c.at();
    c.take(p0, "p0", Nt > MVCAP ? Nt : MVCAP);
    { C o = c.reuse(p0, p0_at, c.at()); o.take(gb, "gb", MVCAP); }
    c.take(tS, "tS", msp);
    c.take(tdl, "tdl", msp);
    c.take(bklo, "bklo", msp);
    c.take(tbl, "tbl", msp);
    c.take(tbh, "tbh", msp);
    c.tail(evolve && cut);
    c.take(llv, "llv", Nt);
    c.take(lpv, "lpv", Nt);
    c.tail(true);
    c.slack("slack", 32);
    bytes = c.size();
  }
  DecideLds() = default;
  PTM_LDS_FN DecideLds(void* base, int Nt, int ms, int WN, bool evolve, bool evb, bool cut) { LdsCarve c(base); carve(c, Nt, ms, WN, evolve, evb, cut); }
};

constexpr int TILE_SCAN_INTS = 257, TILE_SCAN_SLACK = 3 * sizeof(int);

struct Mfma32Lds {
  double* bm;
  double* ptile;
  double* lbox;
  double* red;
  double* gtab = nullptr;
  int* gint = nullptr;
  double* red2 = nullptr;
  double* ebox = nullptr;
  int* tpre = nullptr;
  int* tsum = nullptr;
  size_t bytes;
  template <class C>
  PTM_LDS_FN void carve(C& c, bool gen, bool compacted, int nrung) {
    c.take(bm, "bm", BM_TABLE_DOUBLES);
    c.take(ptile, "ptile", 12 * 64);
    c.take(lbox, "lbox", 64);
    c.take(red, "red", 4 * 128);
    if (gen) {
      c.take(gtab, "gtab", 6 * 32);
      c.take(gint, "gint", 3 * 32);
      c.take(red2, "red2", 4 * 128);
      c.take(ebox, "ebox", 64);
    }
    if (compacted) {
      c.take(tpre, "tpre", nrung);
      c.take(tsum, "tsum", TILE_SCAN_INTS);
      c.slack("slack", TILE_SCAN_SLACK);
    }
    bytes = c.size();
  }
  Mfma32Lds() = default;
  PTM_LDS_FN Mfma32Lds(void* base, bool gen, bool compacted, int nrung) { LdsCarve c(base); carve(c, gen, compacted, nrung); }
};

struct BoxPreLds {
  double* bm;
  double* lbox;
  int* tpre;
  int* pcn;
  int* tsum;
  size_t bytes;
  template <class C>
  PTM_LDS_FN void carve(C& c, int nrung) {
    c.take(bm, "bm", BM_TABLE_DOUBLES);
    c.take(lbox, "lbox", 64);
    c.take(tpre, "tpre", nrung);
    c.take(pcn, "pcn", nrung);
    c.take(tsum, "tsum", TILE_SCAN_INTS);
    c.slack("slack", TILE_SCAN_SLACK);
    bytes = c.size();
  }
  BoxPreLds() = default;
  PTM_LDS_FN BoxPreLds(void* base, int nrung) { LdsCarve c(base); carve(c, nrung); }
};

struct GeneralLds {
  double* bm;
  double* fac = nullptr;
  size_t bytes;
  template <class C>
  PTM_LDS_FN void carve(C& c, bool staged, int prop_stride) {
    c.take(bm, "bm", BM_TABLE_DOUBLES);
    if (staged) c.take(fac, "fac", 4 * prop_stride);
    bytes = c.size();
  }
  GeneralLds() = default;
  PTM_LDS_FN GeneralLds(void* base, bool staged, int prop_stride) { LdsCarve c(base); carve(c, staged, prop_stride); }
};

template <int D, int TILES, int WAVES>
struct MfmaWideLds {
  double* bm;
  double* ptile;
  double* lbox;
  double* red;
  double* lebox;
  size_t bytes;
  template <class C>
  PTM_LDS_FN void carve(C& c) {
    c.take(bm, "bm", BM_TABLE_DOUBLES);
    c.take(ptile, "ptile", TILES * 64);
    c.take(lbox, "lbox", 2 * D);
    c.take(red, "red", WAVES * 64);
    c.take(lebox, "lebox", 2 * D);
    bytes = c.size();
  }
  MfmaWideLds() = default;
  PTM_LDS_FN explicit MfmaWideLds(void* base) { LdsCarve c(base); carve(c); }
};
typedef MfmaWideLds<64, M64_P2_TILES, 4> Mfma64Lds;
typedef MfmaWideLds<128, M128_P2_TILES, M128_THREADS / 64> Mfma128Lds;

}
```

ptmcmc_amd/csrc/ptm_sweep_plan.hpp:

```cpp
#pragma once
#include <cmath>
#include <cstddef>
#include <cstdio>
#include <cstdlib>

namespace ptm {

enum { PLAN_DENSE = 0, PLAN_DIAG = 1, PLAN_LOWER = 2 };

struct SweepFacts {
  int DP, W;
  long long chains;
  int nloc;
  int kind;
  bool has_bounds, bounds_box, all_uniform, has_mean, any_oned;
  int mix_K;
  bool evolving;
  bool tracked;
  bool user_like;
  bool host_prop;
  bool de, ada;
  int mode;
  bool touched;
  bool prior_draw;
  bool history;
};

struct SweepEnv {
  bool force_valu, compact_ok;
  int prefilter;
  int prefilter_grid;
  int de_mfma;
};
inline const SweepEnv& sweep_env() {
  static const SweepEnv v = [] {
    const char* f = getenv("PTM_FORCE_VALU");
    const char* c = getenv("PTM_COMPACT");
    const char* b = getenv("PTM_BOX_PREFILTER");
    const char* g = getenv("PTM_PREFILTER_GRID");
    const char* d = getenv("PTM_DE_MFMA");
    const long gn = (g && *g) ? strtol(g, nullptr, 10) : 0;
    return SweepEnv{f && *f && *f != '0', !(c && *c == '0'), (b && *b) ? (*b == '0' ? -1 : 1) : 0, gn >= 1 ? (int)(gn < (1 << 20) ? gn : (1 << 20)) : 0,
                    (d && *d) ? (*d == '0' ? -1 : 1) : 0};
  }();
  return v;
}

enum SweepFamily { FAM_GENERAL, FAM_LANES, FAM_LANES_ADA, FAM_MFMA32, FAM_MFMA64, FAM_MFMA128 };

struct SweepPlan {
  SweepFamily family;
  int DP, kind;
  bool uni, simple, ada;
  bool gen;
  bool hist;
  int mgen;
  bool ev;
  bool bnd;
  bool compacted;
  bool prefilter;
};
inline bool reads_ladder_major_beta(const SweepPlan& s) { return s.family == FAM_MFMA32 && s.mgen == 0 && s.ev; }

#define PTM_LANES_MAX (1ll << 20)

inline SweepPlan plan_sweep(const SweepFacts& f, const SweepEnv& env) {
  SweepPlan s = {};
  s.DP = f.DP;
  s.kind = f.host_prop ? PLAN_DIAG : f.kind;
  const bool uni = (f.W % 64) == 0;
  const bool ada = f.ada && !f.host_prop;
  const bool box = f.all_uniform && (!f.has_bounds || f.bounds_box);
  const bool recipe = f.has_mean || f.any_oned || f.mix_K != 0;
  const bool plain = !f.has_bounds && f.all_uniform && !recipe && !f.user_like && !ada && !f.evolving && !f.host_prop;
  const bool simple = uni && plain;
  const bool lean_ev = uni && f.evolving && !f.has_bounds && f.all_uniform && !recipe && !f.user_like && !ada && !f.host_prop && !f.tracked;
  const bool mfma_ok = uni && f.mode == 0 && !f.user_like && !f.host_prop && !ada && !env.force_valu;
  const int mk = s.kind == PLAN_DIAG ? PLAN_LOWER : s.kind;

  if (f.DP == 32 && mfma_ok && !f.de) {
    s.family = FAM_MFMA32; s.kind = mk;
    s.compacted = env.compact_ok && f.touched && box && !f.tracked && f.W >= 1024 && f.nloc <= 4096;
    s.hist = f.tracked;
    s.mgen = (simple || lean_ev) ? 0 : !box ? 2 : (s.compacted && !recipe) ? 3 : 1;
    s.ev = !simple && box && f.evolving;
    s.prefilter = env.prefilter >= 0 && s.compacted && s.mgen == 0 && !s.ev && (f.kind == PLAN_LOWER || f.kind == PLAN_DIAG);
    return s;
  }
  if ((f.DP == 64 || f.DP == 128) && mfma_ok && box && !recipe && !f.tracked) {
    s.family = f.DP == 64 ? FAM_MFMA64 : FAM_MFMA128; s.kind = mk;
    s.bnd = f.has_bounds; s.ev = f.evolving;
    return s;
  }
  const long long lanes = f.chains * f.DP;
  const long long lanes_max = f.DP >= 16 ? PTM_LANES_MAX : 4096ll * f.DP, lanes_max_de = f.DP >= 32 ? (1ll << 21) : (1ll << 19);
  if (f.DP >= 64 || f.host_prop ||
      (!env.force_valu && ((!uni && lanes <= lanes_max) || (uni && f.de && f.DP >= 16 && lanes <= lanes_max_de)))) {
    s.family = ada ? FAM_LANES_ADA : FAM_LANES;
    s.gen = !plain;
    return s;
  }
  s.family = FAM_GENERAL;
  s.uni = uni; s.simple = simple; s.ada = ada;
  return s;
}

inline bool de_mfma_applies(const SweepFacts& f, const SweepEnv& env) {
  if (env.de_mfma < 0 || env.force_valu) return false;
  if (f.DP != 32 || (f.W % 64) != 0 || f.mode != 0) return false;
  if (f.user_like || f.host_prop || f.ada) return false;
  if (!f.de || f.prior_draw || f.mix_K <= 0 || !f.history) return false;
  if (!(f.all_uniform && (!f.has_bounds || f.bounds_box))) return false;
  return env.de_mfma > 0 || f.chains * f.DP > (1ll << 21);
}

constexpr int PREFILTER_DIMS = 16;
#ifndef PTM_PREFILTER_THRESHOLD
#define PTM_PREFILTER_THRESHOLD 0.70
#endif
inline void prefilter_sigmas(bool diag, const double* factor, int D, double* sigma) {
  for (int d = 0; d < PREFILTER_DIMS; ++d) {
    double s2 = 0.0;
    if (d < D) {
      if (diag) s2 = factor[d] * factor[d];
      else for (int k = 0; k < D; ++k) s2 += factor[(size_t)d * D + k] * factor[(size_t)d * D + k];
    }
    sigma[d] = std::sqrt(s2);
  }
}
inline double prefilter_out_1d(double sigma, double w) {
  if (!(sigma > 0.0) || !(w < INFINITY)) return 0.0;
  if (!(w > 0.0)) return 1.0;
  const double u = w / sigma, phi0 = 0.3989422804014327;
  const double in = std::erf(u * 0.7071067811865476) - (2.0 / u) * (phi0 - phi0 * std::exp(-0.5 * u * u));
  return in < 0.0 ? 1.0 : (in > 1.0 ? 0.0 : 1.0 - in);
}
inline double prefilter_out_share(const double* sigma, const double* width, int nd) {
  double in = 1.0;
  for (int d = 0; d < nd; ++d) in *= 1.0 - prefilter_out_1d(sigma[d], width[d]);
  return 1.0 - in;
}
inline bool prefilter_flag(const double* sigma, const double* width, int nd, int env_prefilter) {
  if (env_prefilter < 0) return false;
  if (env_prefilter > 0) return true;
  return prefilter_out_share(sigma, width, nd) > PTM_PREFILTER_THRESHOLD;
}

#ifdef __HIPCC__
#define PTM_PLAN_HD __host__ __device__
#else
#define PTM_PLAN_HD
#endif
struct PrefilterSlice { int r, kb, start, nact; };
PTM_PLAN_HD inline PrefilterSlice prefilter_slice(const int* tpre, const int* cnt, int nrung, int ntiles, int tile, int wave) {
  PrefilterSlice s = {0, 0, 0, 0};
  if (tile < 0 || tile >= ntiles) return s;
  int lo = 0, hi = nrung - 1;
  while (lo < hi) { const int mid = (lo + hi) >> 1; if (tpre[mid] > tile) hi = mid; else lo = mid + 1; }
  s.r = lo;
  s.kb = tile - (lo ? tpre[lo - 1] : 0);
  s.start = (s.kb * 4 + wave) * 64;
  const int left = cnt[lo] - s.start;
  s.nact = left <= 0 ? 0 : (left < 64 ? left : 64);
  return s;
}

inline int format_sweep_name(const SweepPlan& s, char* b, size_t n) {
  const auto tf = [](bool v) { return v ? "true" : "false"; };
  switch (s.family) {
    case FAM_MFMA32: return snprintf(b, n, "sweep_mfma32_kernel<%d, %s, %d, %s, %s>", s.kind, tf(s.hist), s.mgen, tf(s.ev), tf(s.compacted));
    case FAM_MFMA64:
    case FAM_MFMA128: return snprintf(b, n, "sweep_mfma%d_kernel<%d, %s, %s>", s.DP, s.kind, tf(s.bnd), tf(s.ev));
    case FAM_LANES: return snprintf(b, n, "sweep_lanes_kernel<%d, %d, %s>", s.DP, s.kind, tf(s.gen));
    case FAM_LANES_ADA: return snprintf(b, n, "sweep_lanes_ada_kernel<%d, %d>", s.DP, s.kind);
    default: break;
  }
  if (s.ada) return snprintf(b, n, "sweep_kernel<%d, %d, %s, false, true>", s.DP, s.kind, tf(s.uni));
  return snprintf(b, n, "sweep_kernel<%d, %d, %s, %s>", s.DP, s.kind, tf(s.uni), tf(s.simple));
}

struct StepFacts {
  int DP, Nt, W;
  bool user_like, host_prop, ada, time_kernels;
  bool evolving, evolve_cut;
  size_t decide_lds;
};
inline bool fused_applies(const StepFacts& f, bool fused_ok) {
  if (!fused_ok || f.DP > 16 || (long long)f.Nt * f.DP > 256 || f.user_like || f.host_prop || f.ada || f.time_kernels) return false;
  if (f.evolving && (f.W > 64 || f.evolve_cut)) return false;
  return f.decide_lds <= 96 * 1024;
}

}
```

ptmcmc_amd/engine.py:

```python
import ctypes as C
import os
import sys

import numpy as np

_HERE = os.path.dirname(os.path.abspath(__file__))
LIB_PATH = os.environ.get("PTM_ENGINE_LIB") or os.path.join(_HERE, "libptm_engine.so")

BOUND_OPEN, BOUND_LIMIT, BOUND_REFLECT, BOUND_WRAP = 0, 1, 2, 3
PRIOR_FLAT, PRIOR_UNIFORM, PRIOR_GAUSSIAN, PRIOR_POLAR, PRIOR_COPOLAR, PRIOR_LOG = 0, 1, 2, 3, 4, 5
PROP_DENSE, PROP_DIAG, PROP_LOWER = 0, 1, 2
ARR_LLIKE, ARR_LPRIOR, ARR_LPOST, ARR_NTRIES, ARR_NACCEPT, ARR_LAST_TYPE, ARR_NHIST, ARR_NSIZE, ARR_ROW_LABELS = range(9)
FN_LOG, FN_EXP, FN_SIN_0_PI, FN_COS_HPI, FN_SQRT, FN_DIV, FN_SQRT_RAW = range(7)
COUNT_MAX = 2**31 - 1
PRIOR_NAMES = {"uni": 1, "uniform": 1, "gauss": 2, "gaussian": 2, "pol": 3, "polar": 3, "cpol": 4, "copol": 4, "log": 5}

EXPORTS = [
    "ptm_last_error", "ptm_abi_version", "ptm_device_count", "ptm_engine_create", "ptm_engine_destroy",
    "ptm_set_bounds", "ptm_set_prior", "ptm_set_target_gaussian", "ptm_set_target_callback", "ptm_set_prior_callback", "ptm_set_ladder", "ptm_set_evolve_temps", "ptm_get_invtemps", "ptm_set_invtemps",
    "ptm_set_proposals", "ptm_set_proposal_rung", "ptm_set_proposal_mixture", "ptm_set_proposal_callback", "ptm_set_proposal_de", "ptm_set_proposal_prior_draw", "ptm_set_states", "ptm_init_from_prior", "ptm_init_from_prior_k", "ptm_draw_prior_rows", "ptm_get_history_chains", "ptm_sweep", "ptm_step", "ptm_sync",
    "ptm_copy_llike", "ptm_copy_lprior", "ptm_llike_device_ptr", "ptm_exchange_decide", "ptm_exchange_decide_gathered", "ptm_set_shard_map", "ptm_exchange_redo_count", "ptm_exchange_redo", "ptm_exchange_finish_and_sweep", "ptm_exchange_install", "ptm_sweep_rungs", "ptm_exchange_buffer_doubles", "ptm_exchange_row_capacity", "ptm_shard_unique_id", "ptm_shard_init", "ptm_shard_step", "ptm_shard_finalize", "ptm_get_states", "ptm_batch_begin", "ptm_batch_end",
    "ptm_get_array", "ptm_get_swap_counts", "ptm_get_last_swaps", "ptm_max_swaps_per_step", "ptm_get_history", "ptm_get_history_invtemps", "ptm_set_history", "ptm_set_map", "ptm_get_map", "ptm_restore", "ptm_step_count",
    "ptm_timer_start", "ptm_timer_stop", "ptm_get_kernel_times", "ptm_calibrate", "ptm_get_counter_sums", "ptm_get_ladder_stats", "ptm_sweep_kernel_name", "ptm_step_kernel_name", "ptm_debug_eval",
    "ptm_debug_philox", "ptm_debug_boxmuller", "ptm_debug_sqrt_scan", "ptm_debug_evaluate",
    "ptm_dev_alloc", "ptm_dev_free", "ptm_dev_copy",
    "ptm_set_target_device", "ptm_target_device_rows", "ptm_get_best_evaluated",
    "ptm_set_proposal_adaptive", "ptm_get_proposal_adapt_state", "ptm_set_proposal_adapt_state",
    "ptm_ess_windowed", "ptm_ess_report", "ptm_ess_series_windowed", "ptm_ess_series_report", "ptm_ess_last_on_device",
    "ptm_log_evidence",
    "ptm_get_prefilter_counts",
]


class PtmConfig(C.Structure):
    _fields_ = [("struct_size", C.c_uint32), ("dim", C.c_int32), ("n_rungs", C.c_int32), ("rung_begin", C.c_int32),
                ("rung_count", C.c_int32), ("n_walkers", C.c_int32), ("seed", C.c_uint64), ("swap_rate", C.c_double),
                ("add_every_n", C.c_int32), ("min_prior", C.c_double), ("device", C.c_int32), ("stream", C.c_void_p),
                ("time_kernels", C.c_int32), ("swap_log_steps", C.c_int32), ("exchange_row_capacity", C.c_int32), ("history_rungs", C.c_int32),
                ("history_capacity", C.c_int32), ("map_rungs", C.c_int32), ("walker_begin", C.c_int32)]


class PtmCalibration(C.Structure):
    _fields_ = [("copy_GBs", C.c_double), ("copy_bytes", C.c_double), ("copy_ms", C.c_double), ("f64_fma_TFs", C.c_double),
                ("fma_ms", C.c_double), ("sclk_MHz", C.c_double), ("compute_units", C.c_int32), ("reserved", C.c_int32)]


class PtmDeParams(C.Structure):
    _fields_ = [("snooker", C.c_double), ("gamma_one_frac", C.c_double), ("reduce_gamma", C.c_double), ("ignore_frac", C.c_double)]


class PtmAdaptiveSet(C.Structure):
    _fields_ = [("K", C.c_int), ("nested", C.c_int), ("K_inner", C.c_int), ("rate", C.c_double), ("rate_inner", C.c_double)]


class PtmError(RuntimeError):
    pass


_lib = None
_dp = C.POINTER(C.c_double)
_i32p = C.POINTER(C.c_int32)
_i64p = C.POINTER(C.c_int64)
_u32p = C.POINTER(C.c_uint32)

LOGLIKE_BATCH_FN = C.CFUNCTYPE(None, C.c_void_p, _dp, C.c_int, C.c_int, _dp)
PROPOSE_BATCH_FN = C.CFUNCTYPE(None, C.c_void_p, C.c_int, C.c_int, _dp, _i32p, _i32p, C.c_uint64, _dp, _dp, _i32p, _i32p)
PROPOSAL_RESULT_FN = C.CFUNCTYPE(None, C.c_void_p, C.c_int, _i32p, _i32p, _i32p)
LOGLIKE_DEVICE_FN = C.CFUNCTYPE(None, C.c_void_p, C.c_void_p, C.c_int, C.c_int, C.c_void_p, C.c_void_p, C.c_void_p)


TORCH_LOADED_FIRST = None


def load():
    global _lib
    if _lib is not None:
        return _lib
    if not os.path.exists(LIB_PATH):
        raise PtmError("HIP engine not built: %s is missing (run `python -c 'import __graft_entry__ as g; g.build()'`)" % LIB_PATH)
    global TORCH_LOADED_FIRST
    TORCH_LOADED_FIRST = "torch" in sys.modules
    L = C.CDLL(LIB_PATH)
    L.ptm_last_error.restype = C.c_char_p
    L.ptm_sweep_kernel_name.restype = C.c_char_p
    L.ptm_sweep_kernel_name.argtypes = [C.c_void_p]
    if hasattr(L, "ptm_step_kernel_name"):
        L.ptm_step_kernel_name.restype = C.c_char_p
        L.ptm_step_kernel_name.argtypes = [C.c_void_p]
    L.ptm_step_count.restype = C.c_uint64
    L.ptm_step_count.argtypes = [C.c_void_p]
    L.ptm_engine_create.argtypes = [C.POINTER(PtmConfig), C.POINTER(C.c_void_p)]
    L.ptm_engine_destroy.argtypes = [C.c_void_p]
    L.ptm_set_bounds.argtypes = [C.c_void_p, _i32p, _i32p, _dp, _dp]
    L.ptm_set_prior.argtypes = [C.c_void_p, _i32p, _dp, _dp]
    L.ptm_set_target_gaussian.argtypes = [C.c_void_p, _dp, _dp, C.c_double]
    L.ptm_set_target_callback.argtypes = [C.c_void_p, C.c_void_p, C.c_void_p]
    if hasattr(L, "ptm_set_prior_callback"):
        L.ptm_set_prior_callback.argtypes = [C.c_void_p, C.c_void_p, C.c_void_p]
    L.ptm_set_ladder.argtypes = [C.c_void_p, _dp]
    L.ptm_set_evolve_temps.argtypes = [C.c_void_p, C.c_double, C.c_double]
    L.ptm_get_invtemps.argtypes = [C.c_void_p, _dp]
    L.ptm_set_invtemps.argtypes = [C.c_void_p, _dp]
    L.ptm_set_proposals.argtypes = [C.c_void_p, C.c_int, _dp, _dp]
    L.ptm_set_states.argtypes = [C.c_void_p, _dp, _dp]
    L.ptm_init_from_prior.argtypes = [C.c_void_p]
    L.ptm_init_from_prior_k.argtypes = [C.c_void_p, C.c_int]
    if hasattr(L, "ptm_draw_prior_rows"):
        L.ptm_draw_prior_rows.argtypes = [C.c_void_p, C.c_int, C.c_int, _dp, _dp, _dp]
    L.ptm_sweep.argtypes = [C.c_void_p, C.c_int]
    L.ptm_step.argtypes = [C.c_void_p, C.c_int]
    L.ptm_sync.argtypes = [C.c_void_p]
    L.ptm_llike_device_ptr.argtypes = [C.c_void_p, C.POINTER(C.c_void_p)]
    L.ptm_exchange_decide.argtypes = [C.c_void_p, C.c_void_p, C.c_void_p, C.c_int, C.c_void_p, C.c_void_p]
    L.ptm_copy_llike.argtypes = [C.c_void_p, C.c_int, C.c_int, C.c_void_p]
    if hasattr(L, "ptm_copy_lprior"):
        L.ptm_copy_lprior.argtypes = [C.c_void_p, C.c_int, C.c_int, C.c_void_p]
        L.ptm_exchange_decide_gathered.argtypes = [C.c_void_p, C.c_void_p, C.c_void_p, C.c_void_p, C.c_void_p]
    if hasattr(L, "ptm_set_shard_map"):
        L.ptm_set_shard_map.argtypes = [C.c_void_p, C.c_int, _i32p, C.c_int]
        L.ptm_exchange_redo_count.argtypes = [C.c_void_p, _i32p]
        L.ptm_exchange_redo.argtypes = [C.c_void_p, C.c_void_p, C.c_void_p, C.c_void_p, C.c_void_p]
    L.ptm_dev_alloc.argtypes = [C.c_size_t, C.POINTER(C.c_void_p)]
    L.ptm_dev_free.argtypes = [C.c_void_p]
    L.ptm_dev_copy.argtypes = [C.c_void_p, C.c_void_p, C.c_size_t]
    L.ptm_exchange_finish_and_sweep.argtypes = [C.c_void_p, C.c_void_p, C.c_void_p]
    L.ptm_exchange_install.argtypes = [C.c_void_p, C.c_void_p, C.c_void_p]
    L.ptm_sweep_rungs.argtypes = [C.c_void_p, C.c_int, C.c_int, C.c_int]
    L.ptm_get_states.argtypes = [C.c_void_p, _dp]
    if hasattr(L, "ptm_batch_begin"):
        L.ptm_batch_begin.argtypes = [C.c_void_p]
        L.ptm_batch_end.argtypes = [C.c_void_p]
    L.ptm_get_array.argtypes = [C.c_void_p, C.c_int, C.c_void_p]
    L.ptm_get_swap_counts.argtypes = [C.c_void_p, _i64p, _i64p]
    L.ptm_get_last_swaps.argtypes = [C.c_void_p, _i32p, _i32p]
    L.ptm_max_swaps_per_step.argtypes = [C.c_void_p]
    L.ptm_timer_start.argtypes = [C.c_void_p]
    L.ptm_timer_stop.argtypes = [C.c_void_p, C.POINTER(C.c_float)]
    L.ptm_get_kernel_times.argtypes = [C.c_void_p, C.POINTER(C.c_float), C.c_int, C.POINTER(C.c_int)]
    L.ptm_calibrate.argtypes = [C.c_void_p, C.POINTER(PtmCalibration)]
    L.ptm_get_counter_sums.argtypes = [C.c_void_p, _i64p, _i64p]
    if hasattr(L, "ptm_get_prefilter_counts"):
        L.ptm_get_prefilter_counts.argtypes = [C.c_void_p, _i64p]
    L.ptm_get_ladder_stats.argtypes = [C.c_void_p, _i64p]
    L.ptm_debug_eval.argtypes = [C.c_int, C.c_int, _dp, _dp, _dp, C.c_int]
    L.ptm_debug_philox.argtypes = [C.c_int, C.c_uint64, C.c_int, C.c_uint32, C.c_uint64, C.c_uint32, _u32p]
    L.ptm_debug_boxmuller.argtypes = [C.c_int, _u32p, _u32p, _dp, _dp, C.c_int]
    L.ptm_exchange_buffer_doubles.argtypes = [C.c_void_p]
    L.ptm_exchange_row_capacity.argtypes = [C.c_void_p]
    L.ptm_get_history.argtypes = [C.c_void_p, _dp, _dp, _dp, _i32p]
    L.ptm_get_history_invtemps.argtypes = [C.c_void_p, _dp]
    L.ptm_set_history.argtypes = [C.c_void_p, _dp, _dp, _dp, _i32p, _dp]
    L.ptm_set_map.argtypes = [C.c_void_p, _dp, _dp, _dp, _dp]
    L.ptm_get_map.argtypes = [C.c_void_p, _dp, _dp, _dp, _dp]
    L.ptm_set_proposal_rung.argtypes = [C.c_void_p, C.c_int, _dp, C.c_double]
    L.ptm_set_proposal_mixture.argtypes = [C.c_void_p, C.c_int, _dp, _dp, _dp]
    L.ptm_set_proposal_de.argtypes = [C.c_void_p, C.POINTER(PtmDeParams), C.c_int, _dp]
    L.ptm_set_proposal_prior_draw.argtypes = [C.c_void_p, C.c_int]
    L.ptm_set_proposal_callback.argtypes = [C.c_void_p, C.c_void_p, C.c_void_p, C.c_void_p]
    L.ptm_shard_unique_id.argtypes = [C.c_void_p]
    L.ptm_shard_init.argtypes = [C.c_void_p, C.c_void_p, C.c_int, C.c_int, _i32p, C.c_int]
    L.ptm_shard_step.argtypes = [C.c_void_p, C.c_int]
    L.ptm_shard_finalize.argtypes = [C.c_void_p]
    L.ptm_restore.argtypes = [C.c_void_p, _dp, _dp, _i32p, _i32p, _i32p, C.POINTER(C.c_int64), C.c_uint64, C.POINTER(C.c_int64),
                              C.POINTER(C.c_int64)]
    L.ptm_debug_sqrt_scan.argtypes = [C.c_int, C.POINTER(C.c_uint64)]
    L.ptm_debug_evaluate.argtypes = [C.c_void_p, _dp, C.c_int, _i32p, _dp, _dp, _dp]
    if hasattr(L, "ptm_set_target_device"):
        L.ptm_set_target_device.argtypes = [C.c_void_p, C.c_void_p, C.c_void_p, C.c_void_p, C.c_void_p]
        L.ptm_target_device_rows.argtypes = [C.c_void_p]
        L.ptm_get_best_evaluated.argtypes = [C.c_void_p, _dp, _dp]
    if hasattr(L, "ptm_set_proposal_adaptive"):
        L.ptm_set_proposal_adaptive.argtypes = [C.c_void_p, C.POINTER(PtmAdaptiveSet), _dp, _dp, _dp, _dp, _i32p, _i32p]
        L.ptm_get_proposal_adapt_state.argtypes = [C.c_void_p, _dp, _dp, _i32p, _i32p]
        L.ptm_set_proposal_adapt_state.argtypes = [C.c_void_p, _dp, _dp, _i32p, _i32p]
    if hasattr(L, "ptm_ess_windowed"):
        L.ptm_ess_windowed.argtypes = [C.c_void_p, C.c_int, C.c_int, C.c_int, C.c_int, C.c_int, _dp, _i32p]
        L.ptm_ess_report.argtypes = [C.c_void_p, C.c_int, C.c_int, C.c_int, C.c_int, C.c_double, _dp, _i32p]
        L.ptm_ess_series_windowed.argtypes = [C.c_int, _dp, C.c_int64, C.c_int, C.c_int, C.c_int, C.c_int, C.c_int, _dp, _i32p]
        L.ptm_ess_series_report.argtypes = [C.c_int, _dp, C.c_int64, C.c_int, C.c_int, C.c_int, C.c_int, C.c_double, _dp, _i32p]
        L.ptm_ess_last_on_device.argtypes = [C.c_void_p]
    if hasattr(L, "ptm_log_evidence"):
        L.ptm_log_evidence.argtypes = [C.c_void_p, C.c_int, _dp, _dp, _dp, _i32p]
    _lib = L
    return L


def _wrap_int32_device(torch, ptr, dev):
    class _Arr:
        __cuda_array_interface__ = {"shape": (1,), "typestr": "<i4", "data": (int(ptr), False), "version": 2}
    return torch.as_tensor(_Arr(), device=dev)


def _chk(rc):
    if rc != 0:
        raise PtmError("ptm error %d: %s" % (rc, load().ptm_last_error().decode()))


def _d(a):
    return a.ctypes.data_as(_dp)


def device_count():
    return load().ptm_device_count()


def debug_eval(fn, a, b=None, device=-1):
    a = np.ascontiguousarray(a, dtype=np.float64)
    bb = a if b is None else np.ascontiguousarray(b, dtype=np.float64)
    out = np.empty_like(a)
    _chk(load().ptm_debug_eval(device, fn, _d(a), _d(bb), _d(out), a.size))
    return out


def debug_philox(seed, tag, stream, step, block, device=-1):
    o = (C.c_uint32 * 4)()
    _chk(load().ptm_debug_philox(device, seed, tag, stream, step, block, o))
    return [int(v) for v in o]


def debug_boxmuller(k1, k2, device=-1):
    k1 = np.ascontiguousarray(k1, dtype=np.uint32)
    k2 = np.ascontiguousarray(k2, dtype=np.uint32)
    z0, z1 = np.empty(k1.size), np.empty(k1.size)
    _chk(load().ptm_debug_boxmuller(device, k1.ctypes.data_as(_u32p), k2.ctypes.data_as(_u32p), _d(z0), _d(z1), k1.size))
    return z0, z1


def debug_sqrt_scan(device=-1):
    n = C.c_uint64()
    _chk(load().ptm_debug_sqrt_scan(device, C.byref(n)))
    return n.value


def _series3(series):
    a = np.ascontiguousarray(series, dtype=np.float64)
    if a.ndim != 3:
        raise ValueError("series must be an array [n, nseries, nfeat]")
    return a


def ess_series_windowed(series, width, every, burn, device=-1):
    a = _series3(series)
    n, ns, nf = a.shape
    ess, nwin = np.empty(ns), np.empty(ns, dtype=np.int32)
    _chk(load().ptm_ess_series_windowed(device, _d(a), n, ns, nf, int(width), int(every), int(burn), _d(ess), nwin.ctypes.data_as(_i32p)))
    return ess, nwin


def effective_samples_series(series, width, every, esslimit=-1, device=-1):
    a = _series3(series)
    n, ns, nf = a.shape
    ess, length = np.empty(ns), np.empty(ns, dtype=np.int32)
    _chk(load().ptm_ess_series_report(device, _d(a), n, ns, nf, int(width), int(every), float(esslimit), _d(ess), length.ctypes.data_as(_i32p)))
    return ess, length


class DeviceBuffer:

    def __init__(self, nbytes):
        p = C.c_void_p()
        _chk(load().ptm_dev_alloc(nbytes, C.byref(p)))
        self.ptr, self.nbytes = p.value, nbytes

    def data_ptr(self):
        return self.ptr

    def copy_from(self, src_ptr, nbytes=None):
        _chk(load().ptm_dev_copy(self.ptr, src_ptr, self.nbytes if nbytes is None else nbytes))

    def to_numpy(self, dtype=np.float64):
        out = np.empty(self.nbytes // np.dtype(dtype).itemsize, dtype=dtype)
        _chk(load().ptm_dev_copy(out.ctypes.data_as(C.c_void_p), self.ptr, self.nbytes))
        return out

    def free(self):
        if self.ptr:
            load().ptm_dev_free(self.ptr)
            self.ptr = None

    __del__ = free

    def slice(self, offset_bytes, nbytes):
        assert 0 <= offset_bytes and offset_bytes + nbytes <= self.nbytes
        return _DeviceView(self, offset_bytes, nbytes)


class _DeviceView:
    def __init__(self, parent, offset, nbytes):
        self.parent, self.ptr, self.nbytes = parent, parent.ptr + offset, nbytes

    def data_ptr(self):
        return self.ptr

    def copy_from(self, src_ptr, nbytes=None):
        _chk(load().ptm_dev_copy(self.ptr, src_ptr, self.nbytes if nbytes is None else nbytes))

    def to_numpy(self, dtype=np.float64):
        out = np.empty(self.nbytes // np.dtype(dtype).itemsize, dtype=dtype)
        _chk(load().ptm_dev_copy(out.ctypes.data_as(C.c_void_p), self.ptr, self.nbytes))
        return out


def geometric_ladder(n_rungs, tmax):
    import math
    tratio = math.exp(math.log(tmax) / (n_rungs - 1)) if n_rungs > 1 else 1.0
    t, beta = 1.0, [1.0]
    for _ in range(1, n_rungs):
        t = t * tratio
        beta.append(1 / t)
    return np.array(beta)


class Engine:

# ... 503 lines not shown
```

Before: 11.61 billion.

## Add f32 box prefilter kernel with conservative per-rung margins

Adds a box-prefilter kernel that runs Box-Muller in f32 using hardware log/sin/cos and does the proposal projection with f32 MFMA. It no longer stages the f64 Box-Muller table in LDS. To keep decisions safe, it widens the box bounds by per-rung margins derived from the proposal factor row sums plus face slack, so f32 error only sends borderline candidates to the exact path. This kernel is the default, and the old f64 kernel stays reachable through an env flag. The risk is that the margin bounds might not fully cover the f32 error, and a debug scan kernel is included to check that.

```diff
diff --git a/include/ptm_engine.h b/include/ptm_engine.h
--- a/include/ptm_engine.h
+++ b/include/ptm_engine.h
@@ -200,6 +200,7 @@
 int ptm_debug_philox(int device, uint64_t seed, int tag, uint32_t stream, uint64_t step, uint32_t block, uint32_t out[4]);
 int ptm_debug_boxmuller(int device, const uint32_t* k1, const uint32_t* k2, double* z0, double* z1, int n);
 int ptm_debug_sqrt_scan(int device, uint64_t* mismatches);
+int ptm_debug_boxmuller_f32_scan(int device, double out[8]);
 int ptm_dev_alloc(size_t bytes, void** out);
 int ptm_dev_free(void* p);
 int ptm_dev_copy(void* dst, const void* src, size_t bytes);
diff --git a/ptmcmc_amd/csrc/ptm_aux_kernels.hpp b/ptmcmc_amd/csrc/ptm_aux_kernels.hpp
--- a/ptmcmc_amd/csrc/ptm_aux_kernels.hpp
+++ b/ptmcmc_amd/csrc/ptm_aux_kernels.hpp
@@ -349,6 +349,34 @@
   if (out) atomicAdd(mismatches + 1, out);
 }
 
+__global__ __launch_bounds__(256) void debug_boxmuller_f32_scan_kernel(int which, unsigned long long* out) {
+  const uint32_t tid = blockIdx.x * blockDim.x + threadIdx.x;
+  const uint32_t stride = gridDim.x * blockDim.x;
+  double worst = 0.0, top = 0.0;
+  unsigned long long nan = 0;
+  for (uint64_t k = tid; k < (1ull << 32); k += stride) {
+    float r, sn, cs;
+    double d;
+    if (which == 0) {
+      boxmuller_f32_parts((uint32_t)k, 0u, r, sn, cs);
+      d = __builtin_fabs((double)r - bm_sqrt(bm_neg2log((uint32_t)k, (const double*)BM_TABLE)));
+      top = __builtin_fabs((double)r) > top ? __builtin_fabs((double)r) : top;
+    } else {
+      double z0, z1;
+      boxmuller_f32_parts(0u, (uint32_t)k, r, sn, cs);
+      boxmuller_finish(1.0, (uint32_t)k, (const double*)BM_TABLE, z0, z1);
+      const double dc = __builtin_fabs((double)cs - z0), ds = __builtin_fabs((double)sn - z1);
+      d = dc > ds ? dc : ds;
+      if (dc != dc || ds != ds) d = dc + ds;
+    }
+    if (d != d) nan++;
+    else worst = d > worst ? d : worst;
+  }
+  atomicMax(out, (unsigned long long)__double_as_longlong(worst));
+  atomicMax(out + 1, (unsigned long long)__double_as_longlong(top));
+  if (nan) atomicAdd(out + 2, nan);
+}
+
 __global__ __launch_bounds__(256) void calib_copy_kernel(const uint4* __restrict__ src, uint4* __restrict__ dst, size_t n16) {
   const size_t stride = (size_t)gridDim.x * blockDim.x;
   for (size_t i = (size_t)blockIdx.x * blockDim.x + threadIdx.x; i < n16; i += stride) dst[i] = src[i];
diff --git a/ptmcmc_amd/csrc/ptm_box_prefilter.hpp b/ptmcmc_amd/csrc/ptm_box_prefilter.hpp
--- a/ptmcmc_amd/csrc/ptm_box_prefilter.hpp
+++ b/ptmcmc_amd/csrc/ptm_box_prefilter.hpp
@@ -178,4 +178,182 @@
   }
 }
 
+#ifndef PTM_BP_F32_WAVES
+#define PTM_BP_F32_WAVES 4
+#endif
+#ifndef PTM_BP_F32_MFMA64
+#define PTM_BP_F32_MFMA64 0
+#endif
+#ifndef PTM_BP_F32_ROWS_AHEAD
+#define PTM_BP_F32_ROWS_AHEAD 0
+#endif
+
+struct BoxPreF32 {
+  BoxPre b;
+  const float* margin;
+};
+
+typedef float bp_f4 __attribute__((ext_vector_type(4)));
+
+struct BpRowsF32 {
+  bp_d2 v0[4], v1[4];
+  bp_f4 mg;
+  double ll, lp, beta, ta[4];
+};
+
+__global__ __launch_bounds__(256, PTM_BP_F32_WAVES) void box_prefilter_f32_kernel(const BoxPreF32 pf) {
+  extern __shared__ __attribute__((aligned(16))) double bp_lds[];
+  const BoxPre& p = pf.b;
+  const int nrung = p.nrung, per = (nrung + 255) / 256;
+  const BoxPreF32Lds L(bp_lds, nrung);
+  const int wave = threadIdx.x >> 6, l = threadIdx.x & 63, q = l >> 4, j = l & 15;
+  if (threadIdx.x < 64) L.lbox[threadIdx.x] = p.box_row[threadIdx.x];
+  int loc = 0;
+  for (int k = 0; k < per; ++k) {
+    const int r = threadIdx.x * per + k;
+    if (r < nrung) { const int n = p.pcnt[p.rung0 + r]; L.pcn[r] = n; loc += (n + 255) >> 8; L.tpre[r] = loc; }
+  }
+  L.tsum[threadIdx.x] = loc;
+  __syncthreads();
+  if (threadIdx.x == 0) { int run = 0; for (int t = 0; t < 256; ++t) { const int v = L.tsum[t]; L.tsum[t] = run; run += v; } L.tsum[256] = run; }
+  __syncthreads();
+  const int off = L.tsum[threadIdx.x];
+  for (int k = 0; k < per; ++k) {
+    const int r = threadIdx.x * per + k;
+    if (r < nrung) L.tpre[r] += off;
+  }
+  __syncthreads();
+  const int ntiles = L.tsum[256];
+  const bp_d2* box = reinterpret_cast<const bp_d2*>(L.lbox) + q;
+  const int wmask = p.labelled ? 0xFFFF : -1;
+  const int G = (int)gridDim.x;
+  const int lt = PTM_BP_F32_MFMA64 ? l : 16 * q + (j >> 2) + 4 * (j & 3);
+
+  auto slice_of = [&](int tile) {
+    PrefilterSlice s = prefilter_slice(L.tpre, L.pcn, nrung, ntiles, tile, wave);
+    s.r = __builtin_amdgcn_readfirstlane(s.r);
+    s.start = __builtin_amdgcn_readfirstlane(s.start);
+    s.nact = __builtin_amdgcn_readfirstlane(s.nact);
+    return s;
+  };
+  auto load_entry = [&](const PrefilterSlice& s) {
+    if (s.nact == 0) return 0;
+    return p.pidx[(size_t)(p.rung0 + s.r) * p.W + s.start + (l < s.nact ? l : s.nact - 1)];
+  };
+  auto load_rows = [&](const PrefilterSlice& s, int mine, BpRowsF32& R) {
+    if (s.nact == 0) return;
+    const int rl = p.rung0 + s.r;
+    const int c = (int)((size_t)rl * p.W) + (mine & wmask);
+    R.ll = p.ll[c]; R.lp = p.lp[c];
+    R.beta = as_c(p.beta)[p.r0 + rl];
+    const double* timg = p.prop_tiles + (size_t)rl * (16 * 64) + lt;
+#pragma unroll
+    for (int sl = 0; sl < 4; ++sl) R.ta[sl] = timg[((0 * 4 + sl) * 2 + 0) * 64];
+    R.mg = reinterpret_cast<const bp_f4*>(pf.margin + (size_t)rl * PREFILTER_DIMS)[q];
+#pragma unroll
+    for (int g = 0; g < 4; ++g) {
+      const int e = __shfl(mine, 16 * g + j, 64);
+      const int slot = p.labelled ? (int)((unsigned int)e >> 16) : rl;
+      const bp_d2* rp = reinterpret_cast<const bp_d2*>(p.x + ((size_t)slot * p.W + (e & wmask)) * 32) + q;
+      R.v0[g] = rp[0];
+      R.v1[g] = rp[4];
+    }
+  };
+
+  constexpr bool RA = PTM_BP_F32_ROWS_AHEAD != 0;
+  constexpr int EA = RA ? 2 : 1;
+  PrefilterSlice sl[EA + 1] = {};
+  int m[EA + 1] = {};
+  BpRowsF32 R[2] = {};
+#pragma unroll
+  for (int k = 0; k < EA; ++k) { sl[k] = slice_of((int)blockIdx.x + k * G); m[k] = load_entry(sl[k]); }
+  if (RA) load_rows(sl[0], m[0], R[0]);
+  uint64_t pbits = 0;
+  int pmine = 0, pbase = 0;
+  size_t plbase = 0;
+  auto flush = [&]() {
+    if (pbits == 0) return;
+    const int base = __builtin_amdgcn_readfirstlane(pbase);
+    if ((pbits >> l) & 1ull) p.cidx[plbase + base + __builtin_popcountll(pbits & ((1ull << l) - 1ull))] = pmine;
+    pbits = 0;
+  };
+  PTM_BP_ARRIVED();
+  unsigned int seen = 0, settled = 0;
+  for (int tile = blockIdx.x; tile < ntiles; tile += G) {
+    sl[EA] = slice_of(tile + EA * G);
+    m[EA] = load_entry(sl[EA]);
+    if (RA) load_rows(sl[1], m[1], R[1]);
+    else load_rows(sl[0], m[0], R[0]);
+    PTM_BP_STAGE();
+    const PrefilterSlice s = sl[0];
+    const int mine = m[0], nact = s.nact;
+    const int rl = p.rung0 + s.r, rg = p.r0 + rl;
+    const size_t lbase = (size_t)rl * p.W;
+    const BpRowsF32& T = R[0];
+    uint64_t inbox = 0;
+    if (nact) {
+      float ta[4];
+#pragma unroll
+      for (int g = 0; g < 4; ++g) {
+        const int wk = __shfl(mine, 16 * g + j, 64) & wmask;
+        const uint32_t stream = (uint32_t)(wk + p.w_off) * (uint32_t)p.Nt + (uint32_t)rg;
+        const u32x4 o = draw_block(p.seed, TAG_MH, stream, p.step, (uint32_t)(1 + q));
+        float z[4];
+        boxmuller_f32(o.v0, o.v1, z[0], z[1]);
+        boxmuller_f32(o.v2, o.v3, z[2], z[3]);
+        if (g == 0) {
+#pragma unroll
+          for (int k = 0; k < 4; ++k) ta[k] = (float)T.ta[k];
+        }
+        const double m0 = (double)T.mg[0], m1 = (double)T.mg[1], m2 = (double)T.mg[2], m3 = (double)T.mg[3];
+        const bp_d2 lo0 = box[0] - bp_d2{m0, m1}, lo1 = box[4] - bp_d2{m2, m3}, hi0 = box[16] + bp_d2{m0, m1}, hi1 = box[20] + bp_d2{m2, m3};
+#if PTM_BP_F32_MFMA64
+        bp_d4 acc = bp_d4{0.0, 0.0, 0.0, 0.0};
+#pragma unroll
+        for (int k = 0; k < 4; ++k) acc = __builtin_amdgcn_mfma_f64_16x16x4f64(T.ta[k], (double)z[k], acc, 0, 0, 0);
+#else
+        bp_f4 acc = bp_f4{0.0f, 0.0f, 0.0f, 0.0f};
+#pragma unroll
+        for (int k = 0; k < 4; ++k) acc = __builtin_amdgcn_mfma_f32_16x16x4f32(ta[k], z[k], acc, 0, 0, 0);
+#endif
+        const double x0 = T.v0[g].x + (double)acc[0], x1 = T.v0[g].y + (double)acc[1], x2 = T.v1[g].x + (double)acc[2], x3 = T.v1[g].y + (double)acc[3];
+        const bool out = (x0 < lo0.x) | (x0 > hi0.x) | (x1 < lo0.y) | (x1 > hi0.y) | (x2 < lo1.x) | (x2 > hi1.x) | (x3 < lo1.y) | (x3 > hi1.y);
+        uint64_t b = __builtin_amdgcn_ballot_w64(!out);
+        b &= b >> 32;
+        b &= b >> 16;
+        inbox |= (b & 0xFFFFull) << (16 * g);
+      }
+    }
+    PTM_BP_STAGE();
+    PTM_BP_ARRIVED();
+    if (nact) {
+      const int c = (int)lbase + (mine & wmask);
+      const double cur_lpost = T.lp + T.beta * T.ll;
+      const bool live = l < nact;
+      const bool finite = __builtin_fabs(cur_lpost) < __builtin_inf();
+      const bool settle = live && finite && ((inbox >> l) & 1ull) == 0;
+      const bool keep = live && !settle;
+      const uint64_t kbits = __builtin_amdgcn_ballot_w64(keep);
+      const int nk = __builtin_popcountll(kbits);
+      flush();
+      if (settle) (void)__hip_atomic_fetch_add(&p.ntries[c], 1, __ATOMIC_RELAXED, __HIP_MEMORY_SCOPE_AGENT);
+      if (nk) {
+        pbits = kbits; pmine = mine; plbase = lbase;
+        const int rlv = __builtin_amdgcn_mov_dpp(rl, 0xE4, 0xF, 0xF, true);
+        if (l == 0) pbase = atomicAdd(&p.ccnt[rlv], nk);
+      }
+      seen += (unsigned int)nact;
+      settled += (unsigned int)(nact - nk);
+    }
+#pragma unroll
+    for (int k = 0; k < EA; ++k) { sl[k] = sl[k + 1]; m[k] = m[k + 1]; }
+    if (RA) R[0] = R[1];
+  }
+  flush();
+  if (l == 0 && seen) {
+    atomicAdd(p.counts, (unsigned long long)seen);
+    if (settled) atomicAdd(p.counts + 1, (unsigned long long)settled);
+  }
 }
+
+}
diff --git a/ptmcmc_amd/csrc/ptm_device_math.hpp b/ptmcmc_amd/csrc/ptm_device_math.hpp
--- a/ptmcmc_amd/csrc/ptm_device_math.hpp
+++ b/ptmcmc_amd/csrc/ptm_device_math.hpp
@@ -268,6 +268,20 @@
   boxmuller_finish(bm_sqrt(bm_neg2log(k1, tab)), k2, tab, z0, z1);
 }
 
+__device__ __forceinline__ void boxmuller_f32_parts(uint32_t k1, uint32_t k2, float& r, float& sn, float& cs) {
+  const float u = ((float)k1 + 0.5f) * 2.3283064365386963e-10f;
+  r = __builtin_sqrtf(__builtin_fmaxf(-1.3862943611198906f * __builtin_amdgcn_logf(u), 0.0f));
+  const float t = ((float)k2 + 0.5f) * 2.3283064365386963e-10f;
+  sn = __builtin_amdgcn_sinf(t);
+  cs = __builtin_amdgcn_cosf(t);
+}
+__device__ __forceinline__ void boxmuller_f32(uint32_t k1, uint32_t k2, float& z0, float& z1) {
+  float r, sn, cs;
+  boxmuller_f32_parts(k1, k2, r, sn, cs);
+  z0 = r * cs;
+  z1 = r * sn;
+}
+
 __device__ __forceinline__ double fmod_det(double x, double w) {
   const double q = __builtin_trunc(x / w);
   double r = __builtin_fma(-q, w, x);
diff --git a/ptmcmc_amd/csrc/ptm_engine.hip b/ptmcmc_amd/csrc/ptm_engine.hip
--- a/ptmcmc_amd/csrc/ptm_engine.hip
+++ b/ptmcmc_amd/csrc/ptm_engine.hip
@@ -120,6 +120,8 @@
   unsigned char *pf_flag = nullptr, *h_pf_flag = nullptr;
   unsigned long long* pf_counts = nullptr;
   std::vector<double> pf_sigma;
+  std::vector<double> pf_margin_nat;
+  float *pf_margin = nullptr, *h_pf_margin = nullptr;
   bool pf_dirty = true;
   int pf_flagged = 0, pf_grid = 0;
   bool touched = false;
@@ -448,7 +450,7 @@
   for (auto& b : e->host_blocks) (void)hipHostFree(b.first);
   void* ptrs[] = {e->xdev, e->rowof, e->ll, e->lp, e->ntries, e->naccept, e->last_type, e->arr_below, e->arr_above, e->mv_src, e->mv_dst, e->mv_n,
                   e->err, e->nhist, e->swap_cnt, e->touch, e->swap_log, e->hist.x, e->hist.ll, e->hist.lp, e->hist.meta, e->map.lpost, e->map.ll, e->map.lp, e->map.x, e->blo,
-                  e->bhi, e->ptype, e->bmin, e->bmax, e->plo, e->phi, e->pcoef, e->P2, e->mean, e->beta, e->prop, e->prop_tiles, e->P2_tiles, e->box_row, e->onedfrac, e->mix, e->beta_w, e->betaC, e->beta_add, e->hist.beta, e->xprop, e->lprior_new, e->llike_new, e->hastings, e->htype, e->hvalid, e->acc_out, e->cidx, e->ccnt, e->pidx, e->pcnt, e->pf_flag, e->pf_counts,
+                  e->bhi, e->ptype, e->bmin, e->bmax, e->plo, e->phi, e->pcoef, e->P2, e->mean, e->beta, e->prop, e->prop_tiles, e->P2_tiles, e->box_row, e->onedfrac, e->mix, e->beta_w, e->betaC, e->beta_add, e->hist.beta, e->xprop, e->lprior_new, e->llike_new, e->hastings, e->htype, e->hvalid, e->acc_out, e->cidx, e->ccnt, e->pidx, e->pcnt, e->pf_flag, e->pf_counts, e->pf_margin,
                   e->pub_x, e->lad_flags, e->lad_prof, e->shard_ends, e->redo_flag, e->sums, e->de_init, e->de_hast, e->de_type,
                   e->ada_leaf, e->ada_dbl, e->ada_int, e->dl_own_x ? e->dl_x : nullptr, e->dl_own_ll ? e->dl_ll : nullptr, e->dl_count, e->dl_rows, e->dl_chunks, e->dl_xprop,
                   e->dl_lprior_new, e->dl_llike_new, e->dl_best, e->ess_ws};
@@ -456,6 +458,7 @@
     if (p) (void)hipFree(p);
   if (e->h_sums) (void)hipHostFree(e->h_sums);
   if (e->h_pf_flag) (void)hipHostFree(e->h_pf_flag);
+  if (e->h_pf_margin) (void)hipHostFree(e->h_pf_margin);
   for (hipEvent_t ev : e->kev) (void)hipEventDestroy(ev);
   if (e->t0) (void)hipEventDestroy(e->t0);
   if (e->t1) (void)hipEventDestroy(e->t1);
@@ -862,7 +865,12 @@
   if ((rc = upload(e->onedfrac, f.data(), (size_t)nloc, e->stream))) return rc;
   e->prop_kind = kind; e->prop_stride = stride; e->have_prop = 1;
   e->pf_sigma.assign((size_t)nloc * PREFILTER_DIMS, 0.0);
-  for (int r = 0; r < nloc; ++r) prefilter_sigmas(kind == PTM_PROP_DIAG, factors + (size_t)r * (kind == PTM_PROP_DIAG ? D : D * D), D, &e->pf_sigma[(size_t)r * PREFILTER_DIMS]);
+  e->pf_margin_nat.assign((size_t)nloc * PREFILTER_DIMS, 0.0);
+  for (int r = 0; r < nloc; ++r) {
+    const double* fr = factors + (size_t)r * (kind == PTM_PROP_DIAG ? D : D * D);
+    prefilter_sigmas(kind == PTM_PROP_DIAG, fr, D, &e->pf_sigma[(size_t)r * PREFILTER_DIMS]);
+    prefilter_margins(kind == PTM_PROP_DIAG, fr, D, &e->pf_margin_nat[(size_t)r * PREFILTER_DIMS]);
+  }
   e->pf_dirty = true;
   return PTM_OK;
 }
@@ -1153,6 +1161,7 @@
     if ((rc = upload(e->prop_tiles + (size_t)local_rung * ntile * 64, tiles.data(), tiles.size(), e->stream))) return rc;
   }
   prefilter_sigmas(kind == PTM_PROP_DIAG, factor, D, &e->pf_sigma[(size_t)local_rung * PREFILTER_DIMS]);
+  prefilter_margins(kind == PTM_PROP_DIAG, factor, D, &e->pf_margin_nat[(size_t)local_rung * PREFILTER_DIMS]);
   e->pf_dirty = true;
   if (one_d_frac >= 0) {
     if (one_d_frac > 1) return fail(PTM_ERR_INVALID, "oneDfrac must be in [0,1]");
@@ -1415,6 +1424,13 @@
     e->pf_flagged += fl[r];
   }
   HIPCHK(hipMemcpyAsync(e->pf_flag, fl, (size_t)e->nloc, hipMemcpyHostToDevice, e->stream));
+  const size_t nm = (size_t)e->nloc * PREFILTER_DIMS;
+  if (!e->h_pf_margin) HIPCHK(hipHostMalloc((void**)&e->h_pf_margin, nm * sizeof(float), hipHostMallocDefault));
+  for (int r = 0; r < e->nloc; ++r)
+    for (int d = 0; d < PREFILTER_DIMS; ++d)
+      e->h_pf_margin[(size_t)r * PREFILTER_DIMS + 4 * (d & 3) + (d >> 2)] = d >= nd ? 0.0f :
+          prefilter_margin_f32((e->pf_margin_nat.size() == nm ? e->pf_margin_nat[(size_t)r * PREFILTER_DIMS + d] : INFINITY) + prefilter_face_slack(e->h_plo[d], e->h_phi[d]));
+  HIPCHK(hipMemcpyAsync(e->pf_margin, e->h_pf_margin, nm * sizeof(float), hipMemcpyHostToDevice, e->stream));
   e->pf_dirty = false;
   return PTM_OK;
 }
@@ -1452,7 +1468,8 @@
     if (pre) {
       if (!e->pidx) {
         int rc;
-        if ((rc = dalloc(&e->pidx, (size_t)e->Nc)) || (rc = dalloc(&e->pcnt, (size_t)e->nloc)) || (rc = dalloc(&e->pf_flag, (size_t)e->nloc)) || (rc = dalloc(&e->pf_counts, 2))) return rc;
+        if ((rc = dalloc(&e->pidx, (size_t)e->Nc)) || (rc = dalloc(&e->pcnt, (size_t)e->nloc)) || (rc = dalloc(&e->pf_flag, (size_t)e->nloc)) || (rc = dalloc(&e->pf_counts, 2)) ||
+            (rc = dalloc(&e->pf_margin, (size_t)e->nloc * PREFILTER_DIMS))) return rc;
         HIPCHK(hipMemsetAsync(e->pf_counts, 0, 16, e->stream));
         e->pf_dirty = true;
       }
@@ -1472,11 +1489,16 @@
       b.seed = e->cfg.seed; b.step = e->step;
       b.x = p.x; b.ll = e->ll; b.lp = e->lp; b.beta = e->beta; b.prop_tiles = e->prop_tiles; b.box_row = e->box_row; b.ntries = e->ntries;
       b.pidx = e->pidx; b.pcnt = e->pcnt; b.cidx = e->cidx; b.ccnt = e->ccnt; b.counts = e->pf_counts;
-      const size_t lds = BoxPreLds(nullptr, nr).bytes;
+      const bool exact = sweep_env().prefilter_exact != 0;
+      BoxPreF32 bf;
+      bf.b = b; bf.margin = e->pf_margin;
+      const size_t lds = exact ? BoxPreLds(nullptr, nr).bytes : BoxPreF32Lds(nullptr, nr).bytes;
       if (!e->pf_grid) {
         int per_cu = 0, dev = 0;
         hipDeviceProp_t pr;
-        if (hipOccupancyMaxActiveBlocksPerMultiprocessor(&per_cu, (const void*)box_prefilter_kernel, 256, BoxPreLds(nullptr, e->nloc).bytes) != hipSuccess || per_cu <= 0) { (void)hipGetLastError(); per_cu = 2; }
+        const hipError_t oc = exact ? hipOccupancyMaxActiveBlocksPerMultiprocessor(&per_cu, (const void*)box_prefilter_kernel, 256, BoxPreLds(nullptr, e->nloc).bytes)
+                                    : hipOccupancyMaxActiveBlocksPerMultiprocessor(&per_cu, (const void*)box_prefilter_f32_kernel, 256, BoxPreF32Lds(nullptr, e->nloc).bytes);
+        if (oc != hipSuccess || per_cu <= 0) { (void)hipGetLastError(); per_cu = 2; }
         HIPCHK(hipGetDevice(&dev));
         HIPCHK(hipGetDeviceProperties(&pr, dev));
         e->pf_grid = per_cu * (pr.multiProcessorCount > 0 ? pr.multiProcessorCount : 256);
@@ -1484,7 +1506,9 @@
         if (cap > 0 && cap < e->pf_grid) e->pf_grid = cap;
       }
       const long long tiles = (long long)nr * ((e->W + 255) / 256);
-      hipLaunchKernelGGL(box_prefilter_kernel, dim3((unsigned)(tiles < e->pf_grid ? tiles : e->pf_grid)), dim3(256), lds, e->stream, b);
+      const dim3 grid((unsigned)(tiles < e->pf_grid ? tiles : e->pf_grid));
+      if (exact) hipLaunchKernelGGL(box_prefilter_kernel, grid, dim3(256), lds, e->stream, b);
+      else hipLaunchKernelGGL(box_prefilter_f32_kernel, grid, dim3(256), lds, e->stream, bf);
       HIPCHK(hipGetLastError());
     }
     p.cidx = e->cidx; p.ccnt = e->ccnt; p.cidx_slot = labelled ? 1 : 0;
@@ -3387,6 +3411,28 @@
   return PTM_OK;
 }
 
+extern "C" int ptm_debug_boxmuller_f32_scan(int device, double out[8]) {
+  int rc = need_device();
+  if (rc) return rc;
+  if (!out) return fail(PTM_ERR_INVALID, "null argument");
+  if (device >= 0) HIPCHK(hipSetDevice(device));
+  unsigned long long* d = nullptr;
+  HIPCHK(hipMalloc((void**)&d, 48));
+  HIPCHK(hipMemset(d, 0, 48));
+  hipLaunchKernelGGL(debug_boxmuller_f32_scan_kernel, dim3(256 * 16), dim3(256), 0, 0, 0, d);
+  hipLaunchKernelGGL(debug_boxmuller_f32_scan_kernel, dim3(256 * 16), dim3(256), 0, 0, 1, d + 3);
+  HIPCHK(hipGetLastError());
+  unsigned long long v[6] = {0, 0, 0, 0, 0, 0};
+  HIPCHK(hipMemcpy(v, d, 48, hipMemcpyDeviceToHost));
+  (void)hipFree(d);
+  double w[6];
+  memcpy(w, v, sizeof w);
+  out[0] = w[0]; out[1] = w[1]; out[2] = (double)v[2];
+  out[3] = w[3]; out[4] = (double)v[5];
+  out[5] = PTM_BP_DZ; out[6] = PTM_BP_F32_SLACK; out[7] = 0.0;
+  return PTM_OK;
+}
+
 extern "C" int ptm_debug_evaluate(ptm_engine* e, const double* X, int n, int32_t* valid, double* Xe, double* lprior, double* llike) {
   if (!e || !X || n < 1) return fail(PTM_ERR_INVALID, "bad argument");
   const size_t D = e->D, DP = e->DP;
diff --git a/ptmcmc_amd/csrc/ptm_lds_layout.hpp b/ptmcmc_amd/csrc/ptm_lds_layout.hpp
--- a/ptmcmc_amd/csrc/ptm_lds_layout.hpp
+++ b/ptmcmc_amd/csrc/ptm_lds_layout.hpp
@@ -188,6 +188,25 @@
   PTM_LDS_FN BoxPreLds(void* base, int nrung) { LdsCarve c(base); carve(c, nrung); }
 };
 
+struct BoxPreF32Lds {
+  double* lbox;
+  int* tpre;
+  int* pcn;
+  int* tsum;
+  size_t bytes;
+  template <class C>
+  PTM_LDS_FN void carve(C& c, int nrung) {
+    c.take(lbox, "lbox", 64);
+    c.take(tpre, "tpre", nrung);
+    c.take(pcn, "pcn", nrung);
+    c.take(tsum, "tsum", TILE_SCAN_INTS);
+    c.slack("slack", TILE_SCAN_SLACK);
+    bytes = c.size();
+  }
+  BoxPreF32Lds() = default;
+  PTM_LDS_FN BoxPreF32Lds(void* base, int nrung) { LdsCarve c(base); carve(c, nrung); }
+};
+
 struct GeneralLds {
   double* bm;
   double* fac = nullptr;
diff --git a/ptmcmc_amd/csrc/ptm_sweep_plan.hpp b/ptmcmc_amd/csrc/ptm_sweep_plan.hpp
--- a/ptmcmc_amd/csrc/ptm_sweep_plan.hpp
+++ b/ptmcmc_amd/csrc/ptm_sweep_plan.hpp
@@ -31,6 +31,7 @@
   int prefilter;
   int prefilter_grid;
   int de_mfma;
+  int prefilter_exact;
 };
 inline const SweepEnv& sweep_env() {
   static const SweepEnv v = [] {
@@ -39,9 +40,10 @@
     const char* b = getenv("PTM_BOX_PREFILTER");
     const char* g = getenv("PTM_PREFILTER_GRID");
     const char* d = getenv("PTM_DE_MFMA");
+    const char* x = getenv("PTM_BOX_PREFILTER_EXACT");
     const long gn = (g && *g) ? strtol(g, nullptr, 10) : 0;
     return SweepEnv{f && *f && *f != '0', !(c && *c == '0'), (b && *b) ? (*b == '0' ? -1 : 1) : 0, gn >= 1 ? (int)(gn < (1 << 20) ? gn : (1 << 20)) : 0,
-                    (d && *d) ? (*d == '0' ? -1 : 1) : 0};
+                    (d && *d) ? (*d == '0' ? -1 : 1) : 0, (x && *x && *x != '0') ? 1 : 0};
   }();
   return v;
 }
@@ -128,6 +130,36 @@
     sigma[d] = std::sqrt(s2);
   }
 }
+#define PTM_BP_DZ 6.0e-4
+#define PTM_BP_F32_SLACK 7.0e-6
+#define PTM_BP_F32_TINY 3.0e-36
+inline double prefilter_margin(double sumabs) {
+  if (sumabs == 0.0) return 0.0;
+  if (!(sumabs <= 1e37)) return INFINITY;
+  return (PTM_BP_DZ + PTM_BP_F32_SLACK) * sumabs + PTM_BP_F32_TINY;
+}
+inline void prefilter_margins(bool diag, const double* factor, int D, double* margin) {
+  for (int d = 0; d < PREFILTER_DIMS; ++d) {
+    double s = 0.0;
+    if (d < D) {
+      if (diag) s = std::fabs(factor[d]);
+      else for (int k = 0; k < D; ++k) s += std::fabs(factor[(size_t)d * D + k]);
+    }
+    margin[d] = prefilter_margin(s);
+  }
+}
+inline double prefilter_face_slack(double lo, double hi) {
+  const double a = std::fabs(lo) < INFINITY ? std::fabs(lo) : 0.0, b = std::fabs(hi) < INFINITY ? std::fabs(hi) : 0.0;
+  return 0x1p-50 * (a > b ? a : b);
+}
+inline float prefilter_margin_f32(double m) {
+  if (!(m > 0.0)) return m == 0.0 ? 0.0f : INFINITY;
+  if (m < 1.17549435e-38) return 1.17549435e-38f;
+  float f = (float)m;
+  if ((double)f < m) f = std::nextafterf(f, INFINITY);
+  return f;
+}
+
 inline double prefilter_out_1d(double sigma, double w) {
   if (!(sigma > 0.0) || !(w < INFINITY)) return 0.0;
   if (!(w > 0.0)) return 1.0;
diff --git a/ptmcmc_amd/engine.py b/ptmcmc_amd/engine.py
--- a/ptmcmc_amd/engine.py
+++ b/ptmcmc_amd/engine.py
@@ -22,7 +22,7 @@
     "ptm_copy_llike", "ptm_copy_lprior", "ptm_llike_device_ptr", "ptm_exchange_decide", "ptm_exchange_decide_gathered", "ptm_set_shard_map", "ptm_exchange_redo_count", "ptm_exchange_redo", "ptm_exchange_finish_and_sweep", "ptm_exchange_install", "ptm_sweep_rungs", "ptm_exchange_buffer_doubles", "ptm_exchange_row_capacity", "ptm_shard_unique_id", "ptm_shard_init", "ptm_shard_step", "ptm_shard_finalize", "ptm_get_states", "ptm_batch_begin", "ptm_batch_end",
     "ptm_get_array", "ptm_get_swap_counts", "ptm_get_last_swaps", "ptm_max_swaps_per_step", "ptm_get_history", "ptm_get_history_invtemps", "ptm_set_history", "ptm_set_map", "ptm_get_map", "ptm_restore", "ptm_step_count",
     "ptm_timer_start", "ptm_timer_stop", "ptm_get_kernel_times", "ptm_calibrate", "ptm_get_counter_sums", "ptm_get_ladder_stats", "ptm_sweep_kernel_name", "ptm_step_kernel_name", "ptm_debug_eval",
-    "ptm_debug_philox", "ptm_debug_boxmuller", "ptm_debug_sqrt_scan", "ptm_debug_evaluate",
+    "ptm_debug_philox", "ptm_debug_boxmuller", "ptm_debug_sqrt_scan", "ptm_debug_boxmuller_f32_scan", "ptm_debug_evaluate",
     "ptm_dev_alloc", "ptm_dev_free", "ptm_dev_copy",
     "ptm_set_target_device", "ptm_target_device_rows", "ptm_get_best_evaluated",
     "ptm_set_proposal_adaptive", "ptm_get_proposal_adapt_state", "ptm_set_proposal_adapt_state",
@@ -164,6 +164,8 @@
     L.ptm_restore.argtypes = [C.c_void_p, _dp, _dp, _i32p, _i32p, _i32p, C.POINTER(C.c_int64), C.c_uint64, C.POINTER(C.c_int64),
                               C.POINTER(C.c_int64)]
     L.ptm_debug_sqrt_scan.argtypes = [C.c_int, C.POINTER(C.c_uint64)]
+    if hasattr(L, "ptm_debug_boxmuller_f32_scan"):
+        L.ptm_debug_boxmuller_f32_scan.argtypes = [C.c_int, C.POINTER(C.c_double)]
     L.ptm_debug_evaluate.argtypes = [C.c_void_p, _dp, C.c_int, _i32p, _dp, _dp, _dp]
     if hasattr(L, "ptm_set_target_device"):
         L.ptm_set_target_device.argtypes = [C.c_void_p, C.c_void_p, C.c_void_p, C.c_void_p, C.c_void_p]
@@ -230,6 +232,12 @@
     n = C.c_uint64()
     _chk(load().ptm_debug_sqrt_scan(device, C.byref(n)))
     return n.value
+
+
+def debug_boxmuller_f32_scan(device=-1):
+    o = (C.c_double * 8)()
+    _chk(load().ptm_debug_boxmuller_f32_scan(device, o))
+    return dict(max_dr=o[0], max_r=o[1], radius_nan=int(o[2]), max_dtrig=o[3], trig_nan=int(o[4]), dz=o[5], f32_slack=o[6])
 
 
 def _series3(series):
```

New measurement: 12.02 billion, median of 6. +3.6%, better.
